# i8run/BigDL

Measured on AMD Instinct MI355X. Metric: images/sec (whole node) ResNet-50 224x224 bf16 at 1/2/4/8 MI355X, higher is better.
Workload: dtype bf16; 1 GPU; model=ResNet-50 v1.5 (BigDL ImageNet builder), global_batch=256, per_gpu_batch=256, image=224, parallelism=dp1, optimizer=SGD momentum 0.9 + L2 1e-4 (one rank: no gradient exchange), hip_graph=False, wgrad_side_stream=True, bucketed_overlap=False, grad_compress=none (no exchange)

## Files before the change

### bigdl_amd/nn/conv.py

```python
import math

import torch
import torch.nn.functional as F

from .. import ops
from ..ops import bn as bnops
from ..ops import conv as cv
from ..ops import conv_fn
from ..ops import side_stream
from .abstractnn import AutogradModule, TensorModule, _t_begin, _t_end
from .init_methods import RandomUniform, Zeros

CL = torch.channels_last
BF16 = torch.bfloat16


def _same_pad(inp, k, s, d=1):
    out = -(-inp // s)
    total = max((out - 1) * s + (k - 1) * d + 1 - inp, 0)
    return total // 2, total - total // 2


class SpatialConvolution(TensorModule):
    def __init__(self, nInputPlane, nOutputPlane, kernelW, kernelH, strideW=1, strideH=1, padW=0, padH=0,
# ... 188 lines not shown
        return y

    def _direct_groups(self):
        return self.nGroup > 1 and self.nInputPlane // self.nGroup <= 16

    def _geo_g(self, ph, pw):
        return [self.strideH, self.strideW, ph, pw, self.dilationH, self.dilationW, self.nGroup]

    def _fwd_gpu_grouped(self, x, ph, pw):
        G = self.nGroup
        cin, cout = self.nInputPlane // G, self.nOutputPlane // G
        if self._direct_groups():
            xf = x.float().contiguous()
            OH = cv.out_size(x.shape[2], self.kernelH, self.strideH, ph, self.dilationH)
            OW = cv.out_size(x.shape[3], self.kernelW, self.strideW, pw, self.dilationW)
            y = xf.new_empty(x.shape[0], self.nOutputPlane, OH, OW)
            ops.native.get().gconv(0, xf, self.weight.float().contiguous(),
                                   self.bias.float().contiguous() if self.bias is not None else None, y,
                                   self._geo_g(ph, pw))
            if self.fuse_relu:
                y.relu_()
            self._xf = xf
            self._geom = (x.shape, ph, pw)
            return y.to(BF16).contiguous(memory_format=CL)
        outs = []
        w = self.weight
        self._x16 = cv.to_nhwc_bf16(x) if x.shape[1] % 8 == 0 else None
        for g in range(G):
            xg = cv.to_nhwc_bf16(x[:, g * cin:(g + 1) * cin].contiguous(memory_format=CL))
            wg = cv.weight_krsc_bf16(w[g * cout:(g + 1) * cout])
            bg = self.bias[g * cout:(g + 1) * cout] if self.bias is not None else None
            outs.append(cv.conv2d_fwd(xg, wg, bg, (self.strideH, self.strideW), (ph, pw),
                                      (self.dilationH, self.dilationW), relu=self.fuse_relu))
        self._geom = (x.shape, ph, pw)
        return torch.cat(outs, dim=1).contiguous(memory_format=CL)

    def updateGradInput(self, input, gradOutput):
        if not self.propagateBack:
            return None
        x = self._nchw(input)
        gy = self._nchw(gradOutput)
        squeeze = x.dim() == 3
        if squeeze:
            x, gy = x.unsqueeze(0), gy.unsqueeze(0)
        H, W = x.shape[2], x.shape[3]
        x, ph, pw, eh, ew = self._prep(x)
        if gy.is_cuda:
            gy = self._relu_mask(gy)
            once = getattr(self, "_dgrad_bn_once", False)
            self._dgrad_bn_once = False
            bn_src = getattr(input, "_bn_bwd", None) if (getattr(self, "_dgrad_bn_ok", False) or once) else None
            if bn_src is not None and not torch.is_tensor(bn_src[4]):
                bn_src = bn_src[:4] + ((input if bn_src[4] else None),)
            gi = self._dgrad_gpu(x, gy, ph, pw, None if (squeeze or eh or ew or self.format != "NCHW") else bn_src)
        else:
            gy = self._relu_mask(gy)
            gi = torch.nn.grad.conv2d_input(x.shape, self.weight, gy.float(), (self.strideH, self.strideW),
                                            (ph, pw), (self.dilationH, self.dilationW), self.nGroup)
        if eh or ew:
            gi = gi[:, :, :H, :W]
            if gi.is_cuda:
                gi = gi.contiguous(memory_format=CL)
        if squeeze:
            gi = gi.squeeze(0)
        return self._fmt_out(gi)

    def _relu_mask(self, gy):
        if not self.fuse_relu:
            return gy
        if gy.is_cuda and gy.dtype == BF16:
            return ops.relu_bwd_gpu(gy.contiguous(memory_format=CL), self.output)
        return gy * (self.output > 0)

    def _dgrad_gpu(self, x, gy, ph, pw, bn_src=None):
        gy16 = gy if (gy.dtype == BF16 and gy.is_contiguous(memory_format=CL)) else gy.to(BF16, memory_format=CL)
        if self.nGroup == 1:
            w16 = self._w16_padded()
            if gy16.shape[1] % 8:
                gy16 = cv.pad_dim(gy16, 1)
                w16 = cv.pad_dim(w16, 0)
            wt = getattr(self, "_wt_cache", None)
            if getattr(self, "_wt_stamp", None) != cv.WT_STAMP[0] or wt is None or \
                    tuple(wt.shape) != (w16.shape[1], w16.shape[2], w16.shape[3], w16.shape[0]):
                wt = cv.transpose_w(w16)
            Cp = w16.shape[1]
            xs = (x.shape[0], Cp, x.shape[2], x.shape[3])
            addend = getattr(self, "_dgrad_addend", None)
            self._dgrad_addend = None
            addend_zm = None
            if isinstance(addend, tuple):
                addend, addend_zm = addend
            if addend is not None and Cp != x.shape[1]:
                raise RuntimeError("dgrad addend requires unpadded channels")
            bn = None
            if bn_src is not None and Cp == x.shape[1]:
                bnmod, bx, bmean, baff, bz = bn_src
                bzm = None
                if bz is not None and bz.dtype == torch.uint8:
                    bz, bzm = None, bz
                bn = {"x": bx, "z": bz, "zm": bzm, "mean": bmean, "aff": baff,
                      "red": bnops.new_stats(Cp, gy16.device)}
            gi = cv.conv2d_dgrad(gy16, wt, xs, (self.strideH, self.strideW), (ph, pw),
                                 (self.dilationH, self.dilationW), addend=addend, bn=bn, addend_zm=addend_zm)
            if Cp != x.shape[1]:
                gi = gi[:, : x.shape[1]].contiguous(memory_format=CL)
            elif bn is not None and bn.get("done"):
                gi._bn_red = (bnmod, bn["red"])
            return gi
        G = self.nGroup
        cin, cout = self.nInputPlane // G, self.nOutputPlane // G
        if self._direct_groups():
            gyf = gy.float().contiguous()
            dx = torch.empty(x.shape[0], self.nInputPlane, x.shape[2], x.shape[3], device=gy.device)
            ops.native.get().gconv(1, dx, self.weight.float().contiguous(), None, gyf, self._geo_g(ph, pw))
            return dx.to(BF16).contiguous(memory_format=CL)
        parts = []
        for g in range(G):
            wg = cv.pad_dim(cv.weight_krsc_bf16(self.weight[g * cout:(g + 1) * cout]), 0)
            gyg = cv.pad_dim(gy16[:, g * cout:(g + 1) * cout].contiguous(memory_format=CL), 1)
            xs = (x.shape[0], wg.shape[1], x.shape[2], x.shape[3])
            gi = cv.conv2d_dgrad(gyg, cv.transpose_w(wg), xs, (self.strideH, self.strideW), (ph, pw),
                                 (self.dilationH, self.dilationW))
            parts.append(gi[:, :cin])
        return torch.cat(parts, dim=1).contiguous(memory_format=CL)

    def backward(self, input, gradOutput):
        side = None if self._frozen else side_stream.stream_for(gradOutput)
        if side is None:
            return super().backward(input, gradOutput)
        t0 = _t_begin(gradOutput)
        self.gradInput = self.updateGradInput(input, gradOutput)
        side_stream.begin(side)
        with torch.cuda.stream(side):
            self.accGradParameters(input, gradOutput)
            self._apply_regularizers()
        side_stream.keep(side, input, gradOutput, self.output, getattr(self, "_x16", None),
                         *(getattr(self, "_xpair", None) or (None,))[:1])
        _t_end(self, t0, "backward_time")
        return self.gradInput

    def accGradParameters(self, input, gradOutput):
        x = self._nchw(input)
        gy = self._nchw(gradOutput)
        if x.dim() == 3:
            x, gy = x.unsqueeze(0), gy.unsqueeze(0)
        x, ph, pw, _, _ = self._prep(x)
        if gy.is_cuda:
            gy = self._relu_mask(gy) if self.fuse_relu and not getattr(self, "_masked_cached", False) else gy
            self._wgrad_gpu(x, gy, ph, pw)
            return
        gy = self._relu_mask(gy).float()
        gw = torch.nn.grad.conv2d_weight(x.float(), self.weight.shape, gy, (self.strideH, self.strideW), (ph, pw),
                                         (self.dilationH, self.dilationW), self.nGroup)
        self.gradWeight.add_(gw, alpha=self.scaleW)
        if self.bias is not None:
            self.gradBias.add_(gy.sum(dim=(0, 2, 3)), alpha=self.scaleB)
# ... 340 lines not shown
```

### bigdl_amd/nn/fusion.py

```python
import os

import torch

from ..utils.table import Table
from .activation import ReLU
from .containers import ConcatTable, Sequential, add_activity
from .conv import SpatialConvolution
from .linear import Linear
from .normalization import BatchNormalization
from .table_ops import CAddTable


_TRAIN_NODE_ATTRS = ("res_src", "pass_index", "fold_fanout", "fold_bn")


def _reset(m):
    from .graph import Graph

    for x in [m] + list(m.flattened_layers()):
        if isinstance(x, Graph) and getattr(x, "_order0", None) is not None:
            x.order = x._order0
            x._order0 = None
        if isinstance(x, Graph):
            for n in x.order:
# ... 132 lines not shown
    while isinstance(m, Sequential) and m.modules and m._residual_plan is None:
        m = m.modules[-1]
    return m


def _fuse_sequential(seq):
    mods = seq.modules
    if (len(mods) == 3 and isinstance(mods[0], ConcatTable) and len(mods[0].modules) == 2
            and isinstance(mods[1], CAddTable) and isinstance(mods[2], ReLU)):
        branch, short = mods[0].modules
        if isinstance(branch, Sequential) and branch.modules and isinstance(branch.modules[-1], BatchNormalization):
            bn = branch.modules[-1]
            if bn.nOutput % 8 == 0:
                bn.fuse_relu = True
                seq._residual_plan = (branch, short, bn)
    for a, b in zip(mods[:-1], mods[1:]):
        if isinstance(a, SpatialConvolution) and isinstance(b, BatchNormalization) and a.nGroup == 1:
            a.emit_stats = True
        elif isinstance(a, BatchNormalization) and isinstance(b, ReLU):
            a.fuse_relu = True
            b.passthrough = True
    for a, b, c in zip(mods[:-2], mods[1:-1], mods[2:]):
        if (_dgrad_bn_enabled() and isinstance(a, BatchNormalization) and a.fuse_relu and isinstance(b, ReLU) and b.passthrough
                and isinstance(c, SpatialConvolution) and c.nGroup == 1):
            c._dgrad_bn_ok = True
        elif isinstance(a, (SpatialConvolution, Linear)) and isinstance(b, ReLU):
            a.fuse_relu = True
            b.passthrough = True
    for a, b, c in zip(mods[:-2], mods[1:-1], mods[2:]):
        _plan_deferred_bn(a, b, c)


DEFER_LEVEL = [int(os.environ.get("BIGDL_BN_DEFER", "1") or 0)]


def _defer_consumer(c):
    from .pooling import SpatialMaxPooling

    if isinstance(c, SpatialConvolution):
        if DEFER_LEVEL[0] < 2:
            return False
        return (c.nGroup == 1 and c.format == "NCHW" and type(c).updateOutput is SpatialConvolution.updateOutput
                and type(c)._wgrad_gpu is SpatialConvolution._wgrad_gpu and c.kernelW == 3 and c.kernelH == 3
                and c.strideW == 1 and c.strideH == 1 and c.dilationW == 1 and c.dilationH == 1)
    return DEFER_LEVEL[0] >= 1 and type(c) is SpatialMaxPooling and c.format == "NCHW"


def _plan_deferred_bn(a, b, c):
    if (isinstance(a, BatchNormalization) and a.fuse_relu and not getattr(a, "_graph_dres", False)
            and isinstance(b, ReLU) and b.passthrough and _defer_consumer(c)):
        a._defer_ok = True


def residual_forward(seq, x):
    branch, short, bn = seq._residual_plan
    concat, add, relu = seq.modules
    res = short.forward(x)
    h = x
    for m in branch.modules[:-1]:
        h = m.forward(h)
    if tuple(res.shape) != tuple(h.shape[:1]) + (bn.nOutput,) + tuple(h.shape[2:]):
        raise ValueError(f"residual block: shortcut output {tuple(res.shape)} does not match the branch output")
    out = bn.updateOutput(h, residual=res)
    bn.output = out
    branch.output = out
    concat.output = Table(out, res)
    add.output = out
    relu.output = out
    seq._res_h = h
    return out


MASKED_ADDEND = [os.environ.get("BIGDL_MASKED_ADDEND", "1") != "0"]


SHORTCUT_BN_RED = [os.environ.get("BIGDL_SHORTCUT_BN_RED", "1") != "0"]


def _native_det():
    from ..ops import native

    return native.deterministic()


def residual_backward(seq, x, gradOutput):
    branch, short, bn = seq._residual_plan
    mods = branch.modules
    first = mods[0]
    can_fold = (isinstance(first, SpatialConvolution) and first.propagateBack and first.nGroup == 1
                and first.format == "NCHW" and first.nInputPlane % 8 == 0)
    masked = None
    zm = getattr(bn, "_zm", None)
    if (MASKED_ADDEND[0] and can_fold and zm is not None and type(short).__name__ == "Identity" and first.strideH == 1
            and first.strideW == 1 and torch.is_tensor(gradOutput) and gradOutput.is_cuda
            and tuple(gradOutput.shape) == tuple(x.shape) and x.dtype == torch.bfloat16):
        dh, _ = bn.backward_fused(seq._res_h, gradOutput, need_dres=False)
        gz = gradOutput
        if gz.dtype != torch.bfloat16 or not gz.is_contiguous(memory_format=torch.channels_last):
            gz = gz.to(torch.bfloat16).contiguous(memory_format=torch.channels_last)
        masked = (gz, zm)
        gs = None
    else:
        sec, sbn = None, None
        if SHORTCUT_BN_RED[0] and isinstance(short, Sequential) and short.modules:
            sbn = short.modules[-1]
            xs = getattr(sbn, "_xin", None)
            xb = getattr(bn, "_xin", None)
            if (isinstance(sbn, BatchNormalization) and sbn.train and not sbn.fuse_relu and xs is not None
                    and xb is not None and xs.is_cuda and xs.shape == xb.shape and xs.stride() == xb.stride()
                    and xs.dtype == torch.bfloat16 and xs.shape[1] % 8 == 0 and not _native_det()):
                from ..ops import bn as bnops

                sec = (xs, sbn.saveMean, bnops.new_stats(xs.shape[1], xs.device))
        dh, dres = bn.backward_fused(seq._res_h, gradOutput, need_dres=True, sec=sec)
        if sec is not None:
            dres._bn_red = (sbn, sec[2])
        gs = short.backward(x, dres)
    bn.gradInput = dh
    fold = masked is not None or (can_fold and gs is not None and gs.dtype == x.dtype and gs.shape == x.shape)
    g = dh
    for i in range(len(mods) - 2, -1, -1):
        inp = mods[i - 1].output if i > 0 else x
        if i == 0 and fold:
            first._dgrad_addend = masked if masked is not None else gs
            first._dgrad_bn_once = _dgrad_bn_enabled()
        g = mods[i].backward(inp, g)
    return g if fold else add_activity(g, gs)


def _graph_users(g):
    users = {}
    for n in g.order:
        for p in n.prevs:
            users.setdefault(p.id, []).append(n)
    return users


def _conv_fusable(n):
    m = n.element
    return (type(m).__name__ in ("SpatialConvolution", "SpatialShareConvolution", "SpatialDilatedConvolution")
            and isinstance(m, SpatialConvolution) and m.nGroup == 1 and m.format == "NCHW")


def _conv_out_shape(conv, x):
    from ..ops.conv import out_size

    N, _, H, W = x.shape
    ph, pw = conv._pads(H, W)
    return (N, conv.nOutputPlane, out_size(H, conv.kernelH, conv.strideH, ph, conv.dilationH),
            out_size(W, conv.kernelW, conv.strideW, pw, conv.dilationW))


def _topo_with_deps(g, extra):
    order, state = [], {}
    for root in list(g.output_nodes) + list(g.inputs_nodes):
        stack = [(root, False)]
        while stack:
            n, done = stack.pop()
            if done:
                if state.get(n.id) != 2:
                    state[n.id] = 2
                    order.append(n)
                continue
            st = state.get(n.id)
            if st == 2:
                continue
            if st == 1:
                raise ValueError("inference fusion created a cycle")
            state[n.id] = 1
            stack.append((n, True))
            for p in reversed(list(n.prevs) + extra.get(n.id, [])):
                if state.get(p.id) != 2:
# ... 154 lines not shown
```

### bigdl_amd/nn/normalization.py

```python
import math
import os

import torch
import torch.nn.functional as F

from .. import ops
from ..ops import bn as bnops
from .abstractnn import AutogradModule, TensorModule, _t_begin, _t_end
from .init_methods import Ones, RandomUniform, Zeros

_ZMASK = os.environ.get("BIGDL_BN_ZMASK", "1") != "0"
_DEFER = [os.environ.get("BIGDL_BN_DEFER", "1") != "0"]
CL = torch.channels_last
BF16 = torch.bfloat16


class BatchNormalization(TensorModule):

    def __init__(self, nOutput, eps=1e-5, momentum=0.1, affine=True, initWeight=None, initBias=None,
                 initGradWeight=None, initGradBias=None, dataFormat="NCHW"):
        super().__init__()
        self.nOutput = nOutput
        self.eps = eps
        self.momentum = momentum
# ... 13 lines not shown
        self.saveStd = None
        self.weightInitMethod = RandomUniform(0.0, 1.0) if affine else None
        self.biasInitMethod = Zeros()
        self.reset()
        if initWeight is not None and affine:
            self.weight.copy_(torch.as_tensor(initWeight))
        if initBias is not None and affine:
            self.bias.copy_(torch.as_tensor(initBias))
        if initGradWeight is not None and affine:
            self.gradWeight.copy_(torch.as_tensor(initGradWeight))
        if initGradBias is not None and affine:
            self.gradBias.copy_(torch.as_tensor(initGradBias))

    def reset(self):
        if self.affine:
            with torch.no_grad():
                self.weightInitMethod.init(self.weight)
                self.biasInitMethod.init(self.bias)
        self.runningMean.zero_()
        self.runningVar.fill_(1.0)

    def setParallism(self, n):
        from ..parallel.sync_bn import make_sync_fn

        self.sync_fn = make_sync_fn() if n and n > 1 else None
        return self

    def _to_nchw(self, x):
        if self.dataFormat == "NHWC" and x.dim() == 4:
            return x.permute(0, 3, 1, 2)
        return x

    def _from_nchw(self, y):
        if self.dataFormat == "NHWC" and y.dim() == 4:
            return y.permute(0, 2, 3, 1)
        return y

    def _gpu_ok(self, x):
        if not x.is_cuda or self.nOutput % 8 != 0:
            return False
        if x.dim() == 4:
            return True
        return x.dim() == 2

    def _prep_gpu(self, x):
        if x.dim() == 4:
            if x.dtype != BF16 or not x.is_contiguous(memory_format=CL):
                x = x.to(BF16, memory_format=CL)
        else:
            if x.dtype != BF16 or not x.is_contiguous():
                x = x.to(BF16).contiguous()
        return x

    def updateOutput(self, input, residual=None):
        if residual is None:
            residual = self.__dict__.pop("_graph_residual", None)
        x = self._to_nchw(input)
        if self._gpu_ok(x):
            stats = getattr(input, "_bn_stats", None) if self.train else None
            x = self._prep_gpu(x)
            res = residual
            if res is not None and (res.dtype != BF16 or res.stride() != x.stride()):
                res = res.to(BF16).contiguous(memory_format=CL if x.dim() == 4 else torch.contiguous_format)
            zm = None
            if self.train and self.fuse_relu and res is not None and x.shape[1] % 8 == 0 and _ZMASK:
                zm = torch.empty(x.numel() // 8, dtype=torch.uint8, device=x.device)
            if (self.train and self.fuse_relu and res is None and getattr(self, "_defer_ok", False) and _DEFER[0]
                    and x.dim() == 4 and self.dataFormat == "NCHW"):
                sm, si, aff = bnops.bn_prepare_gpu(x, self.weight, self.bias, self.runningMean, self.runningVar,
                                                   self.eps, self.momentum, stats=stats, sync_fn=self.sync_fn)
                self.saveMean, self.saveStd = sm, si
                self._aff, self._zm, self._xin = aff, None, x
                y = bnops.deferred(x, aff)
                y._bn_bwd = (self, x, sm, aff, False)
                return y
            y, sm, si, aff = bnops.bn_forward_gpu(x, self.weight, self.bias, self.runningMean, self.runningVar,
                                                   self.eps, self.momentum, self.train, stats=stats, res=res,
                                                   relu=self.fuse_relu, sync_fn=self.sync_fn if self.train else None,
                                                   zm=zm)
            self.saveMean, self.saveStd = sm, si
            self._aff = aff if (self.fuse_relu and res is None) else None
            self._zm = zm
            self._xin = x
            if self.train and self.fuse_relu:
                y._bn_bwd = (self, x, sm, self._aff, zm if zm is not None else res is not None)
            return self._from_nchw(y)
        xf = x.float()
        y, mean, invstd = bnops.bn_forward_cpu(xf, self.weight, self.bias, self.runningMean, self.runningVar, self.eps,
                                               self.momentum, self.train,
                                               sync_fn=self.sync_fn if self.train else None)
        if residual is not None:
            y = y + residual.float()
        if self.fuse_relu:
            y = torch.relu(y)
        self.saveMean, self.saveStd = mean, invstd
        self._xin = xf
        return self._from_nchw(y.to(input.dtype) if input.is_floating_point() else y)

    def _direct_grads(self):
        return (not self._frozen) and self.affine and self.scaleW == 1.0 and self.scaleB == 1.0

    def backward_fused(self, input, gradOutput, need_dres=False, sec=None):
        gz = self._to_nchw(gradOutput)
        x = self._xin
        if gz.dtype != BF16 or gz.stride() != x.stride():
            gz = gz.to(BF16).contiguous(memory_format=CL if x.dim() == 4 else torch.contiguous_format)
        aff = getattr(self, "_aff", None)
        zm = getattr(self, "_zm", None)
        z = self._to_nchw(self.output) if (self.fuse_relu and aff is None and zm is None) else None
        direct = self._direct_grads()
        dg = self.gradWeight if direct else (torch.zeros_like(self.runningMean) if self.affine else None)
        db = self.gradBias if direct else (torch.zeros_like(self.runningMean) if self.affine else None)
        pre = getattr(gradOutput, "_bn_red", None)
        red = pre[1] if (pre is not None and pre[0] is self and self.train) else None
        graph_res = getattr(self, "_graph_dres", False)
        dx, dres = bnops.bn_backward_gpu(gz, z, x, self.saveMean, self.saveStd, self.weight, dg, db,
                                         training=self.train, need_dres=need_dres or graph_res,
                                         sync_fn=self.sync_fn if self.train else None, aff=aff, red=red, zm=zm,
                                         sec=sec)
        if graph_res:
            self._dres = dres
        if not direct and self.affine and not self._frozen:
            self.gradWeight.add_(dg, alpha=self.scaleW)
            self.gradBias.add_(db, alpha=self.scaleB)
        return self._from_nchw(dx), dres

    def backward(self, input, gradOutput):
        t0 = _t_begin(gradOutput)
        x = self._to_nchw(input)
        if self._gpu_ok(x):
            self.gradInput, _ = self.backward_fused(input, gradOutput)
        else:
            self.gradInput = self.updateGradInput(input, gradOutput)
            if not self._frozen:
                self.accGradParameters(input, gradOutput)
        _t_end(self, t0, "backward_time")
        return self.gradInput

    def _cpu_grads(self, gradOutput):
# ... 183 lines not shown
```

### bigdl_amd/ops/bn.py

```python
import os
import torch

from . import native


def _P(x):
    return x.numel() // x.shape[1]


def stat_slots():
    return native.get().STAT_SLOTS


class _StatsArena:

    def __init__(self):
        self.buf, self.off, self.active, self.need = None, 0, False, 0

    def begin(self, device):
        if self.need and (self.buf is None or self.buf.numel() < self.need or self.buf.device != device):
            self.buf = torch.empty(self.need, dtype=torch.float32, device=device)
        if self.buf is not None:
            if self.buf.is_cuda and int(os.environ.get("BIGDL_NATIVE_FILL", "7")) & 2:
                native.get().fill_bytes(self.buf, 0)
            else:
                self.buf.zero_()
        self.off, self.need, self.active = 0, 0, True

    def end(self):
        self.active = False

    def take(self, n, device):
        n_al = (n + 63) // 64 * 64
        self.need += n_al
        if self.active and self.buf is not None and self.buf.device == device and self.off + n_al <= self.buf.numel():
            t = self.buf[self.off:self.off + n]
            self.off += n_al
            return t
        t = torch.empty(n, dtype=torch.float32, device=device)
        if t.is_cuda:
            native.get().fill_bytes(t, 0)
            return t
        return t.zero_()


ARENA = _StatsArena()


def new_stats(C, device):
    return ARENA.take(stat_slots() * 2 * C, torch.device(device))


def _reduce_slots_for_sync(buf, C, P, sync_fn):
    red = torch.empty(2 * C, dtype=torch.float32, device=buf.device)
    native.get().bn_slot_reduce(buf, stat_slots(), C, red)
    P = sync_fn(red, P)
    return red, 1, P


def bn_forward_gpu(x, gamma, beta, rmean, rvar, eps, momentum, training, stats=None, res=None, relu=False,
                   out=None, sync_fn=None, zm=None):
    C = x.shape[1]
    P = _P(x)
    C_ = native.get()
    dev = x.device
    if out is None:
        out = torch.empty_like(x)
    aff = torch.empty(2 * C, dtype=torch.float32, device=dev)
    scale, shift = aff[:C], aff[C:]
    smean = torch.empty(C, dtype=torch.float32, device=dev)
    sinv = torch.empty(C, dtype=torch.float32, device=dev)
    nslots = stat_slots()
    Ptot = P
    if training:
        if stats is None:
            stats = new_stats(C, dev)
            C_.bn_stats(x, stats, P, C)
        if sync_fn is not None:
            stats, nslots, Ptot = _reduce_slots_for_sync(stats, C, P, sync_fn)
    else:
        stats, nslots = scale, 0
    C_.bn_finalize(stats, nslots, gamma, beta, rmean, rvar, smean, sinv, scale, shift, Ptot, C, float(eps),
                   float(momentum), bool(training))
    C_.bn_apply(x, scale, shift, res, out, P, C, bool(relu), zm)
    return out, smean, sinv, aff


def bn_prepare_gpu(x, gamma, beta, rmean, rvar, eps, momentum, stats=None, sync_fn=None):
    C = x.shape[1]
    P = _P(x)
    C_ = native.get()
    dev = x.device
    aff = torch.empty(2 * C, dtype=torch.float32, device=dev)
    smean = torch.empty(C, dtype=torch.float32, device=dev)
    sinv = torch.empty(C, dtype=torch.float32, device=dev)
    nslots, Ptot = stat_slots(), P
    if stats is None:
        stats = new_stats(C, dev)
        C_.bn_stats(x, stats, P, C)
    if sync_fn is not None:
        stats, nslots, Ptot = _reduce_slots_for_sync(stats, C, P, sync_fn)
    C_.bn_finalize(stats, nslots, gamma, beta, rmean, rvar, smean, sinv, aff[:C], aff[C:], Ptot, C, float(eps),
                   float(momentum), True)
    return smean, sinv, aff


def deferred(x, aff):
    y = x.detach()
    y._bn_pre = aff
    return y


def materialize(t):
    aff = getattr(t, "_bn_pre", None)
    if aff is None:
        return t
    C = t.shape[1]
    y = torch.empty_like(t)
    native.get().bn_apply(t, aff[:C], aff[C:], None, y, _P(t), C, True)
    return y


def bn_backward_gpu(dz, z, x, smean, sinv, gamma, dgamma, dbeta, training=True, need_dres=False, need_dx=True,
                    sync_fn=None, aff=None, red=None, zm=None, sec=None):
    C = x.shape[1]
    P = _P(x)
    C_ = native.get()
    nslots, Ptot = 0, P
    if not training:
        red = None
    elif red is None:
        red = new_stats(C, x.device)
        C_.bn_bwd_reduce(dz, z, x, smean, red, P, C, aff, zm)
    if training:
        nslots = stat_slots()
        if sync_fn is not None:
            red, nslots, Ptot = _reduce_slots_for_sync(red, C, P, sync_fn)
    coef = torch.empty(3 * C, dtype=torch.float32, device=x.device)
    dx = torch.empty_like(x) if need_dx else None
    dres = torch.empty_like(x) if need_dres else None
    if sec is not None and dres is not None and training:
        x2, mean2, red2 = sec
        C_.bn_bwd_apply(dz, z, x, smean, sinv, gamma, red, nslots, coef, dx, dres, dgamma, dbeta, Ptot, C, aff, zm,
                        x2=x2, mean2=mean2, red2=red2)
    else:
        C_.bn_bwd_apply(dz, z, x, smean, sinv, gamma, red, nslots, coef, dx, dres, dgamma, dbeta, Ptot, C, aff, zm)
    return dx, dres


def bn_forward_cpu(x, gamma, beta, rmean, rvar, eps, momentum, training, sync_fn=None):
    dims = [0] + list(range(2, x.dim()))
    shape = [1, -1] + [1] * (x.dim() - 2)
    if training:
        n = x.numel() // x.shape[1]
        if sync_fn is not None:
            buf = torch.cat([x.sum(dim=dims), (x * x).sum(dim=dims)]).double()
            n = sync_fn(buf, n)
            C = x.shape[1]
            mean = (buf[:C] / n).float()
            var = (buf[C:] / n - (buf[:C] / n) ** 2).clamp_min(0).float()
        else:
            mean = x.mean(dim=dims)
            var = x.var(dim=dims, unbiased=False)
        if rmean is not None:
            unb = var * n / max(n - 1, 1)
            rmean.mul_(1 - momentum).add_(momentum * mean)
            rvar.mul_(1 - momentum).add_(momentum * unb)
    else:
        mean, var = rmean, rvar
    invstd = torch.rsqrt(var + eps)
    xhat = (x - mean.view(shape)) * invstd.view(shape)
    y = xhat
# ... 25 lines not shown
```

### bigdl_amd/ops/conv.py

```python
import os
import torch
import torch.nn.functional as F

from . import native

CL = torch.channels_last
BF16 = torch.bfloat16


def out_size(inp, k, s, p, d=1, ceil=False):
    eff = d * (k - 1) + 1
    num = inp + 2 * p - eff
    if ceil:
        o = -(-num // s) + 1
        if (o - 1) * s >= inp + p:
            o -= 1
        return o
    return num // s + 1


def to_nhwc_bf16(x, cpad=8):
    N, C, H, W = x.shape
    Cp = -(-C // cpad) * cpad
    if x.dtype == BF16 and Cp == C and x.is_contiguous(memory_format=CL):
# ... 56 lines not shown
        native.get().bn_stats(dense, stats, N * OH * OW, K)
        return (out, mat) if pre is not None else out
    mat = native.get().conv_nt(x, w16, out, bias, stats, geo, _fwd_taps(R, S, ph, pw, dh, dw), relu, addend, pre=pre)
    return (out, mat) if pre is not None else out


_TAP_CACHE = {}


def _fwd_taps(R, S, ph, pw, dh, dw):
    key = ("f", R, S, ph, pw, dh, dw)
    t = _TAP_CACHE.get(key)
    if t is None:
        t = []
        for r in range(R):
            for s in range(S):
                t += [r * dh - ph, s * dw - pw, r * S + s]
        _TAP_CACHE[key] = t
    return t


def _fwd_geo(N, H, W, C, OH, OW, sh, sw, ldw, K):
    return [N, H, W, C, OH, OW, sh, sw, ldw, K, K, OH, OW, 1, 1, 0, 0]


def dgrad_phases(H, W, R, S, stride, pad, dil):
    sh, sw = stride
    ph, pw = pad
    dh, dw = dil
    key = ("d", H, W, R, S, sh, sw, ph, pw, dh, dw)
    res = _TAP_CACHE.get(key)
    if res is not None:
        return res
    res = []
    for a in range(sh):
        for b in range(sw):
            nI, nJ = -(-(H - a) // sh), -(-(W - b) // sw)
            if nI <= 0 or nJ <= 0:
                continue
            taps = []
            for r in range(R):
                if (a + ph - r * dh) % sh:
                    continue
                for s in range(S):
                    if (b + pw - s * dw) % sw:
                        continue
                    taps += [(a + ph - r * dh) // sh, (b + pw - s * dw) // sw, r * S + s]
            if taps:
                res.append((a, b, nI, nJ, taps))
    _TAP_CACHE[key] = res
    return res


def conv2d_dgrad(dy, w16t, x_shape, stride, pad, dil=(1, 1), out=None, addend=None, bn=None, addend_zm=None):
    N, C, H, W = x_shape
    _, K, OH, OW = dy.shape
    R, S = w16t.shape[1], w16t.shape[2]
    phases = dgrad_phases(H, W, R, S, stride, pad, dil)
    covered = sum(nI * nJ for (_, _, nI, nJ, _) in phases)
    if addend is not None and not addend.is_contiguous(memory_format=CL):
        addend = addend.contiguous(memory_format=CL)
    if out is None:
        out = torch.empty((N, C, H, W), dtype=BF16, device=dy.device, memory_format=CL)
    if addend_zm is not None and (addend is None or covered != H * W):
        raise ValueError("conv2d_dgrad: a masked addend needs an addend and a data gradient that covers every pixel")
    if covered != H * W:
        mask = 0
        for (a, b, _, _, _) in phases:
            mask |= 1 << (a * stride[1] + b)
        if (out.is_contiguous(memory_format=CL) and C % 8 == 0 and stride[0] * stride[1] <= 32
                and int(os.environ.get("BIGDL_NATIVE_FILL", "7")) & 4):
            native.get().dgrad_fill(out, addend, stride[0], stride[1], mask)
        elif addend is not None:
            out.copy_(addend)
        else:
            out.zero_()
    C_ = native.get()
    ldw = R * S * K
    bnk = {}
    if bn is not None and (covered == H * W or addend is None) and bn["x"].shape == out.shape \
            and bn["x"].stride() == out.stride() and not native.deterministic():
        bnk = dict(bn_x=bn["x"], bn_z=bn["z"], bn_mean=bn["mean"], bn_aff=bn["aff"], bn_red=bn["red"],
                   bn_zm=bn.get("zm"))
        bn["done"] = True
    for (a, b, nI, nJ, taps) in phases:
        geo = [N, OH, OW, K, nI, nJ, 1, 1, ldw, C, C, H, W, stride[0], stride[1], a, b]
        C_.conv_nt(dy, w16t, out, None, None, geo, taps, False, addend, addend_zm=addend_zm, **bnk)
    return out


WT_STAMP = [0]
_DESC_CACHE = {}
DESC_BUILDS = [0]


def prepare_dgrad_weights(convs):
    WT_STAMP[0] += 1
    rows, mods, tile = [], [], 0
    for m in convs:
        if not getattr(m, "_w16_managed", False):
            continue
        wf = getattr(m, "weight", None)
        if wf is None or wf.dim() != 4 or wf.shape[0] % 8 or wf.shape[1] % 8:
            continue
        w16 = m._w16_padded()
        K, C, R, S = w16.shape
        if K % 8 or C % 8 or not w16.is_cuda or not w16.is_contiguous(memory_format=CL):
            continue
        if mods and w16.device != mods[0]._wt_cache.device:
            continue
        wt = getattr(m, "_wt_cache", None)
        if wt is None or tuple(wt.shape) != (C, R, S, K) or wt.device != w16.device:
            wt = torch.empty((C, R, S, K), dtype=BF16, device=w16.device)
            m._wt_cache = wt
        rows.append((w16.data_ptr(), wt.data_ptr(), K, R * S, C, tile))
        tile += ((C + 31) // 32) * ((K + 31) // 32) * R * S
        mods.append(m)
    if not rows:
        return 0
    key = tuple(rows)
    desc = _DESC_CACHE.get(key)
    if desc is None:
        if torch.cuda.is_current_stream_capturing():
            return 0
        if len(_DESC_CACHE) > 8:
            _DESC_CACHE.clear()
        desc = torch.tensor(rows, dtype=torch.int64).to(mods[0]._wt_cache.device)
        _DESC_CACHE[key] = desc
        DESC_BUILDS[0] += 1
    native.get().transpose_krsc_batched(desc, len(rows), tile)
    for m in mods:
        m._wt_stamp = WT_STAMP[0]
    return len(rows)


def end_dgrad_weights():
    WT_STAMP[0] += 1


def transpose_w(w16, out=None):
# ... 149 lines not shown
```

### csrc/batchnorm.hip

```cpp
#include "common.h"
#include "kernels.h"
#include <stdlib.h>

#define STAT_SLOTS BIGDL_STAT_SLOTS

namespace {

template <int MODE, int U>
__global__ __launch_bounds__(256) void chan_reduce_kernel(const bf16_t* __restrict__ x, const bf16_t* __restrict__ dz,
                                                          const bf16_t* __restrict__ z, const float* __restrict__ mean,
                                                          float* __restrict__ out, long P, int C, long rows_per_block,
                                                          const float* __restrict__ aff, const uint8_t* __restrict__ zm) {
  __shared__ float sm[256 * 16];
  const int G = C >> 3;
  const int tid = threadIdx.x;
  const long rbeg = blockIdx.x * rows_per_block;
  const long rend = min(P, rbeg + rows_per_block);
  for (int gbase = 0; gbase < G; gbase += 256) {
    const int gcount = min(256, G - gbase);
    const int rpi = 256 / gcount;
    const int g = gbase + tid % gcount, rsub = tid / gcount;
    float a1[8], a2[8], mu[8], sc[8], sh[8];
#pragma unroll
    for (int e = 0; e < 8; ++e) { a1[e] = 0.f; a2[e] = 0.f; mu[e] = 0.f; sc[e] = 0.f; sh[e] = 0.f; }
// ... 50 lines not shown
              a1[2 * e] += dl; a1[2 * e + 1] += dh;
              a2[2 * e] += dl * (xl - mu[2 * e]);
              a2[2 * e + 1] += dh * (xh - mu[2 * e + 1]);
            }
          }
        }
      }
    }
#pragma unroll
    for (int e = 0; e < 8; ++e) { sm[tid * 16 + e] = a1[e]; sm[tid * 16 + 8 + e] = a2[e]; }
    __syncthreads();
    for (int w = tid; w < gcount * 16; w += 256) {
      const int gg = w >> 4, slot = w & 15;
      float t = 0.f;
      for (int rs = 0; rs < rpi; ++rs) t += sm[(rs * gcount + gg) * 16 + slot];
      const int ch = (gbase + gg) * 8 + (slot & 7);
      atomicAdd(out + (size_t)(blockIdx.x & (STAT_SLOTS - 1)) * 2 * C + (slot < 8 ? 0 : C) + ch, t);
    }
    __syncthreads();
  }
}

int bn_unroll() {
  static int u = [] {
    const char* e = getenv("BIGDL_BN_UNROLL");
    const int v = e ? atoi(e) : 4;
    return (v == 1 || v == 2 || v == 8) ? v : 4;
  }();
  return u;
}

__device__ __forceinline__ void slot_sums(const float* __restrict__ red, int nslots, int C, int c, int sl, double& s1,
                                          double& s2) {
  s1 = 0.0;
  s2 = 0.0;
  for (int k = sl; k < nslots; k += 32) {
    s1 += red[(size_t)k * 2 * C + c];
    s2 += red[(size_t)k * 2 * C + C + c];
  }
#pragma unroll
  for (int o = 16; o > 0; o >>= 1) {
    s1 += __shfl_xor(s1, o, 64);
    s2 += __shfl_xor(s2, o, 64);
  }
}

__global__ void bn_finalize_kernel(const float* __restrict__ stats, int nslots, const float* __restrict__ gamma,
                                   const float* __restrict__ beta, float* run_mean, float* run_var, float* save_mean,
                                   float* save_invstd, float* scale, float* shift, long P, int C, float eps,
                                   float momentum, int training) {
  const int lane = threadIdx.x & 63, sl = lane & 31;
  const int c = (blockIdx.x * (blockDim.x >> 6) + (threadIdx.x >> 6)) * 2 + (lane >> 5);
  if (c >= C) return;
  float mean, invstd;
  if (training) {
    double s1, s2;
    slot_sums(stats, nslots, C, c, sl, s1, s2);
    if (sl != 0) return;
    mean = (float)(s1 / (double)P);
    const float var = fmaxf((float)(s2 / (double)P - (double)mean * mean), 0.f);
    invstd = rsqrtf(var + eps);
    save_mean[c] = mean;
    save_invstd[c] = invstd;
    if (run_mean) {
      const float unbiased = P > 1 ? var * (float)P / (float)(P - 1) : var;
      run_mean[c] = momentum * mean + (1.f - momentum) * run_mean[c];
      run_var[c] = momentum * unbiased + (1.f - momentum) * run_var[c];
    }
  } else {
    if (sl != 0) return;
    mean = run_mean[c];
    invstd = rsqrtf(run_var[c] + eps);
    if (save_mean) { save_mean[c] = mean; save_invstd[c] = invstd; }
  }
  const float g = gamma ? gamma[c] : 1.f, b = beta ? beta[c] : 0.f;
  scale[c] = g * invstd;
  shift[c] = b - mean * g * invstd;
}

template <int U>
__global__ __launch_bounds__(256) void bn_apply_kernel(const bf16_t* __restrict__ x, const float* __restrict__ scale,
                                                       const float* __restrict__ shift, const bf16_t* __restrict__ res,
                                                       bf16_t* __restrict__ y, long P, int C, long rpb, int relu,
                                                       uint8_t* __restrict__ zm) {
  const int G = C >> 3;
  const int gbase = blockIdx.y * 256;
  const int gcount = min(256, G - gbase);
  const int rpi = 256 / gcount;
  const int g = gbase + threadIdx.x % gcount, rsub = threadIdx.x / gcount;
  if (rsub >= rpi) return;
  const long rbeg = blockIdx.x * rpb, rend = min(P, rbeg + rpb);
  const int c0 = g * 8;
  const v4f s0 = *reinterpret_cast<const v4f*>(scale + c0), s1 = *reinterpret_cast<const v4f*>(scale + c0 + 4);
  const v4f b0 = *reinterpret_cast<const v4f*>(shift + c0), b1 = *reinterpret_cast<const v4f*>(shift + c0 + 4);
  const float sc[8] = {s0[0], s0[1], s0[2], s0[3], s1[0], s1[1], s1[2], s1[3]};
  const float sh[8] = {b0[0], b0[1], b0[2], b0[3], b1[0], b1[1], b1[2], b1[3]};
  for (long r0 = rbeg + rsub; r0 < rend; r0 += (long)U * rpi) {
    v4u vx[U], vr[U];
#pragma unroll
    for (int u = 0; u < U; ++u) {
      const long r = r0 + (long)u * rpi;
      const long i = (r < rend ? r : rbeg) * G + g;
      vx[u] = reinterpret_cast<const v4u*>(x)[i];
      vr[u] = v4u{0u, 0u, 0u, 0u};
      if (res) vr[u] = reinterpret_cast<const v4u*>(res)[i];
    }
#pragma unroll
    for (int u = 0; u < U; ++u) {
      const long r = r0 + (long)u * rpi;
      v4u o;
#pragma unroll
      for (int e = 0; e < 4; ++e) {
        float l = lo_bf(vx[u][e]) * sc[2 * e] + sh[2 * e];
        float h = hi_bf(vx[u][e]) * sc[2 * e + 1] + sh[2 * e + 1];
        if (res) { l += lo_bf(vr[u][e]); h += hi_bf(vr[u][e]); }
        if (relu) { l = fmaxf(l, 0.f); h = fmaxf(h, 0.f); }
        o[e] = pack2bf(l, h);
      }
      if (r < rend) {
        reinterpret_cast<v4u*>(y)[r * G + g] = o;
        if (zm) zm[r * G + g] = (uint8_t)bf_to_mask8(o);
      }
    }
  }
}

__global__ void bn_bwd_coeff_kernel(const float* __restrict__ red, int nslots, const float* __restrict__ mean,
                                    const float* __restrict__ invstd, const float* __restrict__ gamma,
                                    float* __restrict__ coef, float* dgamma, float* dbeta, long P, int C, int training) {
  const int lane = threadIdx.x & 63, sl = lane & 31;
  const int c = (blockIdx.x * (blockDim.x >> 6) + (threadIdx.x >> 6)) * 2 + (lane >> 5);
  if (c >= C) return;
  double sdy = 0.0, sdyx = 0.0;
  if (training) slot_sums(red, nslots, C, c, sl, sdy, sdyx);
  if (sl != 0) return;
  const float is = invstd[c];
  const float g = gamma ? gamma[c] : 1.f;
  float A = g * is, B = 0.f, D = 0.f;
  if (training) {
    const float mdy = (float)(sdy / (double)P);
    const float mdyx = (float)(sdyx / (double)P) * is;
    B = -g * is * is * mdyx;
    D = g * is * (mean[c] * is * mdyx - mdy);
    if (dgamma) dgamma[c] += (float)sdyx * is;
    if (dbeta) dbeta[c] += (float)sdy;
  }
  coef[c] = A; coef[C + c] = B; coef[2 * C + c] = D;
}

__global__ void bn_slot_reduce_kernel(const float* __restrict__ in, int nslots, int C, float* __restrict__ out) {
  const int c = blockIdx.x * blockDim.x + threadIdx.x;
  if (c >= 2 * C) return;
  float t = 0.f;
  for (int k = 0; k < nslots; ++k) t += in[(size_t)k * 2 * C + c];
  out[c] = t;
}

__device__ __forceinline__ void load8(const float* p, float* v) {
  const v4f a = *reinterpret_cast<const v4f*>(p), b = *reinterpret_cast<const v4f*>(p + 4);
  v[0] = a[0]; v[1] = a[1]; v[2] = a[2]; v[3] = a[3]; v[4] = b[0]; v[5] = b[1]; v[6] = b[2]; v[7] = b[3];
}

template <int U, bool R2>
__global__ __launch_bounds__(256) void bn_bwd_apply_kernel(const bf16_t* __restrict__ dz, const bf16_t* __restrict__ z,
                                                           const bf16_t* __restrict__ x, const float* __restrict__ coef,
                                                           bf16_t* __restrict__ dx, bf16_t* __restrict__ dres, long P,
                                                           int C, long rpb, const float* __restrict__ aff,
                                                           const uint8_t* __restrict__ zm, const bf16_t* __restrict__ x2,
                                                           const float* __restrict__ mean2, float* __restrict__ red2) {
  const int G = C >> 3;
  const bool xmask = z == nullptr && zm == nullptr && aff != nullptr;
  const __amdgpu_buffer_rsrc_t rzm = __builtin_amdgcn_make_buffer_rsrc(
      const_cast<uint8_t*>(zm), (short)0, zm ? (int)min(P * C / 8, 0x7fffffffl) : 0, 0x00020000);
  const bf16_t* zp = (z && !zm) ? z : x;
  const int gbase = blockIdx.y * 256;
  const int gcount = min(256, G - gbase);
  const int rpi = 256 / gcount;
  const int g = gbase + threadIdx.x % gcount, rsub = threadIdx.x / gcount;
  if (!R2 && rsub >= rpi) return;
  const long rbeg = blockIdx.x * rpb, rend = rsub < rpi ? min(P, rbeg + rpb) : rbeg;
  const int c0 = g * 8;
  float A[8], B[8], D[8], S[8], T[8], M2[8], a1[8], a2[8];
  load8(coef + c0, A);
  load8(coef + C + c0, B);
  load8(coef + 2 * C + c0, D);
  if (xmask) {
    load8(aff + c0, S);
    load8(aff + C + c0, T);
  }
  if (R2) {
    load8(mean2 + c0, M2);
#pragma unroll
    for (int e = 0; e < 8; ++e) { a1[e] = 0.f; a2[e] = 0.f; }
  }
  for (long r0 = rbeg + rsub; r0 < rend; r0 += (long)U * rpi) {
    v4u vd[U], vz[U], vx[U], vx2[U];
    unsigned zb[U];
#pragma unroll
    for (int u = 0; u < U; ++u) {
      const long r = r0 + (long)u * rpi;
      const long i = (r < rend ? r : rbeg) * G + g;
      vd[u] = reinterpret_cast<const v4u*>(dz)[i];
      zb[u] = __builtin_amdgcn_raw_buffer_load_b8(rzm, (unsigned)i, 0, 0);
      vz[u] = reinterpret_cast<const v4u*>(zp)[i];
      vx[u] = reinterpret_cast<const v4u*>(x)[i];
      if (R2) vx2[u] = reinterpret_cast<const v4u*>(x2)[i];
    }
#pragma unroll
    for (int u = 0; u < U; ++u)
      vz[u] = zm ? mask8_to_bf(zb[u]) : z ? vz[u] : v4u{0xffffffffu, 0xffffffffu, 0xffffffffu, 0xffffffffu};
#pragma unroll
    for (int u = 0; u < U; ++u) {
      const long r = r0 + (long)u * rpi;
// ... 56 lines not shown
}

int grid_for(long work, int per_block, int cap) {
  long g = (work + per_block - 1) / per_block;
  if (g > cap) g = cap;
  if (g < 1) g = 1;
  return (int)g;
}

void launch_reduce(int mode, const bf16_t* x, const bf16_t* dz, const bf16_t* z, const float* mean, float* out, long P,
                   int C, hipStream_t st, const float* aff = nullptr, const uint8_t* zm = nullptr) {
  const int G = C >> 3;
  const int rpi = 256 / (G < 256 ? G : 256);
  long blocks = (P + rpi * 16 - 1) / (rpi * 16);
  if (blocks > 2048) blocks = 2048;
  if (bigdl_deterministic() && blocks > 2 * STAT_SLOTS) blocks = 2 * STAT_SLOTS;
  if (blocks < 1) blocks = 1;
  const long rpb = (P + blocks - 1) / blocks;
  blocks = (P + rpb - 1) / rpb;
#define BN_RED(M, U) chan_reduce_kernel<M, U><<<(int)blocks, 256, 0, st>>>(x, dz, z, mean, out, P, C, rpb, aff, zm)
  if (mode == 0) { aff = nullptr; zm = nullptr; }
  switch (bn_unroll()) {
    case 1: if (mode == 0) BN_RED(0, 1); else BN_RED(1, 1); break;
    case 2: if (mode == 0) BN_RED(0, 2); else BN_RED(1, 2); break;
    case 8: if (mode == 0) BN_RED(0, 8); else BN_RED(1, 8); break;
    default: if (mode == 0) BN_RED(0, 4); else BN_RED(1, 4); break;
  }
#undef BN_RED
}

}

extern "C" {

void bigdl_bn_stats(const uint16_t* x, float* stats, long P, int C, hipStream_t st) {
  launch_reduce(0, x, nullptr, nullptr, nullptr, stats, P, C, st);
  HIP_LAUNCH_CHECK();
}

void bigdl_bn_finalize(const float* stats, int nslots, const float* gamma, const float* beta, float* run_mean,
                       float* run_var, float* save_mean, float* save_invstd, float* scale, float* shift, long P, int C,
                       float eps, float momentum, int training, hipStream_t st) {
  bn_finalize_kernel<<<(C + 7) / 8, 256, 0, st>>>(stats, nslots, gamma, beta, run_mean, run_var, save_mean,
                                                   save_invstd, scale, shift, P, C, eps, momentum, training);
  HIP_LAUNCH_CHECK();
}

void bigdl_bn_slot_reduce(const float* in, int nslots, int C, float* out, hipStream_t st) {
  bn_slot_reduce_kernel<<<(2 * C + 255) / 256, 256, 0, st>>>(in, nslots, C, out);
  HIP_LAUNCH_CHECK();
}

void bigdl_bn_apply(const uint16_t* x, const float* scale, const float* shift, const uint16_t* res, uint16_t* y,
                    long P, int C, int relu, hipStream_t st, uint8_t* zm) {
  long rpb = 0;
  const dim3 grid = stationary_grid(P, C, &rpb);
  switch (bn_unroll()) {
    case 1: bn_apply_kernel<1><<<grid, 256, 0, st>>>(x, scale, shift, res, y, P, C, rpb, relu, zm); break;
    case 2: bn_apply_kernel<2><<<grid, 256, 0, st>>>(x, scale, shift, res, y, P, C, rpb, relu, zm); break;
    case 8: bn_apply_kernel<8><<<grid, 256, 0, st>>>(x, scale, shift, res, y, P, C, rpb, relu, zm); break;
    default: bn_apply_kernel<4><<<grid, 256, 0, st>>>(x, scale, shift, res, y, P, C, rpb, relu, zm); break;
  }
  HIP_LAUNCH_CHECK();
}

void bigdl_bn_bwd_reduce(const uint16_t* dz, const uint16_t* z, const uint16_t* x, const float* mean, float* red,
                         long P, int C, const float* aff, hipStream_t st, const uint8_t* zm) {
  launch_reduce(1, x, dz, z, mean, red, P, C, st, aff, zm);
  HIP_LAUNCH_CHECK();
}

void bigdl_bn_bwd_apply(const uint16_t* dz, const uint16_t* z, const uint16_t* x, const float* mean,
                        const float* invstd, const float* gamma, const float* red, int nslots, float* coef,
                        uint16_t* dx, uint16_t* dres, float* dgamma, float* dbeta, long P, int C, int training,
                        const float* aff, hipStream_t st, const uint8_t* zm, const uint16_t* x2u,
                        const float* mean2, float* red2) {
  const bf16_t* x2 = reinterpret_cast<const bf16_t*>(x2u);
  bn_bwd_coeff_kernel<<<(C + 7) / 8, 256, 0, st>>>(red, nslots, mean, invstd, gamma, coef, dgamma, dbeta, P, C,
                                                    training);
  if (dx || dres) {
    long rpb = 0;
    const dim3 grid = stationary_grid(P, C, &rpb);
    if (red2) {
#define BWD2(UU) bn_bwd_apply_kernel<UU, true><<<grid, 256, 0, st>>>(dz, z, x, coef, dx, dres, P, C, rpb, aff, zm, x2, mean2, red2)
      switch (bn_unroll()) {
        case 1: BWD2(1); break;
        case 2: BWD2(2); break;
        case 8: BWD2(8); break;
        default: BWD2(4); break;
      }
#undef BWD2
    } else {
#define BWD1(UU) bn_bwd_apply_kernel<UU, false><<<grid, 256, 0, st>>>(dz, z, x, coef, dx, dres, P, C, rpb, aff, zm, nullptr, nullptr, nullptr)
      switch (bn_unroll()) {
        case 1: BWD1(1); break;
        case 2: BWD1(2); break;
        case 8: BWD1(8); break;
        default: BWD1(4); break;
      }
#undef BWD1
    }
  }
  HIP_LAUNCH_CHECK();
}

}
```

### csrc/bindings.cpp

```cpp
#include <torch/extension.h>
#include <ATen/hip/HIPContext.h>
#include <vector>
#include <algorithm>
#include "kernels.h"

namespace {

using at::Tensor;
using OptT = c10::optional<Tensor>;

hipStream_t stream() { return at::hip::getCurrentHIPStream().stream(); }

void check(const Tensor& t, at::ScalarType dt, const char* name) {
  TORCH_CHECK(t.is_cuda(), name, " must be a GPU tensor");
  TORCH_CHECK(t.scalar_type() == dt, name, " has dtype ", t.scalar_type(), ", expected ", dt);
}
const uint16_t* cbf(const Tensor& t, const char* n) { check(t, at::kBFloat16, n); return (const uint16_t*)t.data_ptr(); }
uint16_t* mbf(const Tensor& t, const char* n) { check(t, at::kBFloat16, n); return (uint16_t*)t.data_ptr(); }
const float* cf(const Tensor& t, const char* n) { check(t, at::kFloat, n); return (const float*)t.data_ptr(); }
float* mf(const Tensor& t, const char* n) { check(t, at::kFloat, n); return (float*)t.data_ptr(); }
const uint16_t* ocbf(const OptT& t, const char* n) { return (t && t->defined()) ? cbf(*t, n) : nullptr; }
uint16_t* ombf(const OptT& t, const char* n) { return (t && t->defined()) ? mbf(*t, n) : nullptr; }
const float* ocf(const OptT& t, const char* n) { return (t && t->defined()) ? cf(*t, n) : nullptr; }
float* omf(const OptT& t, const char* n) { return (t && t->defined()) ? mf(*t, n) : nullptr; }
uint8_t* omzm(const OptT& t, int64_t P, int64_t C, const char* n) {
  if (!(t && t->defined())) return nullptr;
  check(*t, at::kByte, n);
  TORCH_CHECK(t->is_contiguous() && t->numel() == P * (C / 8), n, ": sign mask must be a contiguous [P][C/8] uint8 tensor");
  return (uint8_t*)t->data_ptr();
}

OptT conv_nt(const Tensor& src, const Tensor& wt, const Tensor& out, const OptT& bias, const OptT& stats,
             std::vector<int64_t> geo, std::vector<int64_t> taps, bool relu, const OptT& addend, const OptT& bn_x,
             const OptT& bn_z, const OptT& bn_mean, const OptT& bn_aff, const OptT& bn_red, bool accumulate,
             const OptT& bn_zm, const OptT& addend_zm, const OptT& pre) {
  TORCH_CHECK(geo.size() == 17 || geo.size() == 18, "conv_nt: bad geometry");
  if (stats && stats->defined())
    TORCH_CHECK(stats->numel() >= BIGDL_STAT_SLOTS * 2 * geo[9], "conv_nt: stats must hold STAT_SLOTS x 2Ncol");
  TORCH_CHECK(taps.size() % 3 == 0 && !taps.empty() && taps.size() / 3 <= CONV_MAX_TAPS, "conv_nt: bad taps");
  TORCH_CHECK(!bigdl_deterministic() || (!(stats && stats->defined()) && !(bn_red && bn_red->defined())),
              "conv_nt: epilogue statistics are not deterministic; use bn_stats in deterministic mode");
  ConvArgs a;
  a.src = cbf(src, "src"); a.wt = cbf(wt, "wt");
  a.out = nullptr; a.out32 = nullptr; a.accum32 = accumulate ? 1 : 0;
  if (out.scalar_type() == at::kFloat) a.out32 = mf(out, "out");
  else a.out = mbf(out, "out");
  a.bias = ocf(bias, "bias"); a.stats = omf(stats, "stats");
  a.addend = ocbf(addend, "addend");
  if (a.addend) TORCH_CHECK(addend->numel() == out.numel(), "conv_nt: addend must match out");
  a.bnx = ocbf(bn_x, "bn_x"); a.bnz = ocbf(bn_z, "bn_z"); a.bnmean = ocf(bn_mean, "bn_mean");
  a.bnaff = ocf(bn_aff, "bn_aff"); a.bnred = omf(bn_red, "bn_red");
  a.addzm = nullptr;
  if (addend_zm && addend_zm->defined()) {
    TORCH_CHECK(a.addend && geo[10] == geo[9] && geo[9] % 8 == 0, "conv_nt: a masked addend needs ldo == Ncol");
    a.addzm = omzm(addend_zm, out.numel() / geo[9], geo[9], "addend_zm");
  }
  a.bnzm = nullptr;
  if (bn_zm && bn_zm->defined()) {
    TORCH_CHECK(geo[10] == geo[9] && geo[9] % 8 == 0, "conv_nt: a sign-mask z needs a dense output (ldo == Ncol)");
    a.bnzm = omzm(bn_zm, out.numel() / geo[9], geo[9], "bn_zm");
  }
  if (a.bnred) {
    TORCH_CHECK(a.bnx && a.bnmean && bn_x->numel() == out.numel(), "conv_nt: bn_x must match out, bn_mean required");
    TORCH_CHECK(!a.bnz || bn_z->numel() == out.numel(), "conv_nt: bn_z must match out");
    TORCH_CHECK(bn_mean->numel() >= geo[9] && (!a.bnaff || bn_aff->numel() >= 2 * geo[9]), "conv_nt: bn vectors");
    TORCH_CHECK(bn_red->numel() >= BIGDL_STAT_SLOTS * 2 * geo[9], "conv_nt: bn_red must hold STAT_SLOTS x 2Ncol");
  }
  a.Nb = geo[0]; a.Hs = geo[1]; a.Ws = geo[2]; a.Cs = geo[3]; a.OH = geo[4]; a.OW = geo[5];
  a.mul_h = geo[6]; a.mul_w = geo[7]; a.ldw = geo[8]; a.Ncol = geo[9]; a.ldo = geo[10];
  a.OHo = geo[11]; a.OWo = geo[12]; a.omul_h = geo[13]; a.omul_w = geo[14]; a.ooff_h = geo[15]; a.ooff_w = geo[16];
  a.pstride = geo.size() == 18 ? (int)geo[17] : 0;
  TORCH_CHECK(a.pstride >= 0 && a.pstride % 8 == 0, "conv_nt: pixel stride must be a multiple of 8");
  a.pre = ocf(pre, "pre");
  if (a.pre)
    TORCH_CHECK(pre->numel() >= 2 * geo[3] && a.pstride == 0 && src.numel() % geo[3] == 0 &&
                    (src.is_contiguous() || src.is_contiguous(at::MemoryFormat::ChannelsLast)),
                "conv_nt: pre must hold 2 x Cs floats for a dense source");
  a.ntaps = (int)(taps.size() / 3);
  a.Kdim = a.ntaps * a.Cs;
  a.M = a.Nb * a.OH * a.OW;
  a.ident_out = (a.OHo == a.OH && a.OWo == a.OW && a.omul_h == 1 && a.omul_w == 1 && a.ooff_h == 0 && a.ooff_w == 0);
  a.relu = relu ? 1 : 0;
  int max_tk = 0;
  for (int t = 0; t < a.ntaps; ++t) {
    a.tap_h[t] = (short)taps[3 * t]; a.tap_w[t] = (short)taps[3 * t + 1]; a.tap_k[t] = (short)taps[3 * t + 2];
    max_tk = std::max(max_tk, (int)a.tap_k[t]);
  }
  if (a.pstride > 0) {
    int max_tw = 0;
    for (int t = 0; t < a.ntaps; ++t) max_tw = std::max(max_tw, (int)a.tap_w[t]);
    TORCH_CHECK(((int64_t)(a.OW - 1) * a.mul_w + max_tw) * a.pstride + a.Cs <= (int64_t)a.Ws * a.pstride,
                "conv_nt: a window crosses its source row");
    TORCH_CHECK(src.numel() >= (int64_t)a.Nb * a.Hs * a.Ws * a.pstride, "conv_nt: src too small");
  } else {
    TORCH_CHECK(src.numel() >= (int64_t)a.Nb * a.Hs * a.Ws * a.Cs, "conv_nt: src too small");
  }
  TORCH_CHECK(wt.numel() >= (int64_t)(a.Ncol - 1) * a.ldw + (int64_t)(max_tk + 1) * a.Cs, "conv_nt: weight too small");
  const int64_t out_avail = (int64_t)(out.storage().nbytes() / out.element_size()) - out.storage_offset();
  TORCH_CHECK(a.ldo >= a.Ncol && out_avail >= ((int64_t)a.Nb * a.OHo * a.OWo - 1) * a.ldo + a.Ncol,
              "conv_nt: out too small");
  if (a.addend) TORCH_CHECK(a.ldo == a.Ncol, "conv_nt: an addend needs a dense output (ldo == Ncol)");
  TORCH_CHECK((a.OH - 1) * a.omul_h + a.ooff_h < a.OHo && (a.OW - 1) * a.omul_w + a.ooff_w < a.OWo,
              "conv_nt: output placement out of range");
  OptT materialised;
  if (a.pre && !bigdl_conv_pre_applies(&a)) {
    Tensor y = at::empty_like(src);
    const int64_t P = src.numel() / a.Cs;
    bigdl_bn_apply(a.src, a.pre, a.pre + a.Cs, nullptr, (uint16_t*)y.data_ptr(), P, a.Cs, 1, stream(), nullptr);
    a.src = (const uint16_t*)y.data_ptr();
    a.pre = nullptr;
    materialised = y;
  }
  a.ws = nullptr;
  Tensor ws;
  const long wsn = bigdl_conv_nt_plan(&a);
  if (wsn > 0) {
    ws = at::empty({wsn}, out.options().dtype(at::kFloat));
    a.ws = ws.data_ptr<float>();
  }
  const int rc = bigdl_conv_nt(&a, stream());
  TORCH_CHECK(rc == 0, "conv_nt: unsupported shape (channels must be a multiple of 8; fp32 output needs Ncol % 8 "
              "== 0 and no fused stats / BN / ReLU / addend)");
  return materialised;
}

void conv_wgrad(const Tensor& dy, const Tensor& src, const Tensor& dw, const OptT& dbias, std::vector<int64_t> geo,
                const OptT& pre) {
  TORCH_CHECK(geo.size() == 18, "conv_wgrad: bad geometry");
  WgradArgs a;
  a.dy = cbf(dy, "dy"); a.src = cbf(src, "src"); a.dw = mf(dw, "dw"); a.dbias = omf(dbias, "dbias");
  int* f = &a.Nb;
  for (int i = 0; i < 18; ++i) f[i] = (int)geo[i];
  a.m_per_split = 0;
  a.ws = nullptr;
  a.splits = 0;
  a.pre = ocf(pre, "pre");
  Tensor det_ws;
  a.det_ws = nullptr;
  if (bigdl_deterministic() && a.dbias) {
    det_ws = at::empty({(int64_t)BIGDL_DET_SLOTS * a.Ncol}, dw.options().dtype(at::kFloat));
    a.det_ws = det_ws.data_ptr<float>();
  }
  Tensor mat;
  if (a.pre) {
    TORCH_CHECK(pre->numel() >= 2 * a.Cs && src.numel() % a.Cs == 0, "conv_wgrad: pre must hold 2 x Cs floats");
    if (!bigdl_wgrad_pre_applies(&a)) {
      mat = at::empty_like(src);
      bigdl_bn_apply(a.src, a.pre, a.pre + a.Cs, nullptr, (uint16_t*)mat.data_ptr(), src.numel() / a.Cs, a.Cs, 1,
                     stream(), nullptr);
      a.src = (const uint16_t*)mat.data_ptr();
      a.pre = nullptr;
    }
  }
  TORCH_CHECK(dw.numel() >= (int64_t)a.Ncol * a.Kdim, "conv_wgrad: dw too small");
  TORCH_CHECK(a.M == a.Nb * a.OH * a.OW, "conv_wgrad: M mismatch");
  TORCH_CHECK(dy.numel() >= (int64_t)(a.M - 1) * a.ldy + a.Ncol, "conv_wgrad: dy too small");
  TORCH_CHECK(src.numel() >= (int64_t)a.Nb * a.Hs * a.Ws * a.Cs, "conv_wgrad: src too small");
  Tensor ws;
  const long wsn = bigdl_conv_wgrad_plan(&a);
  if (wsn > 0) {
    ws = at::empty({wsn}, dw.options().dtype(at::kFloat));
    a.ws = ws.data_ptr<float>();
  }
  const int rc = bigdl_conv_wgrad(&a, stream());
  TORCH_CHECK(rc == 0, "conv_wgrad: unsupported shape (channels must be a multiple of 8)");
}

bool conv_wgrad_uses_p8(std::vector<int64_t> geo, bool bias) {
  TORCH_CHECK(geo.size() == 18, "conv_wgrad_uses_p8: bad geometry");
  WgradArgs a{};
  int* f = &a.Nb;
  for (int i = 0; i < 18; ++i) f[i] = (int)geo[i];
  static float dummy;
  a.dbias = bias ? &dummy : nullptr;
  return bigdl_conv_wgrad_uses_p8(&a) != 0;
}

void transpose_krsc(const Tensor& w, const Tensor& wt, int64_t K, int64_t RS, int64_t C) {
  TORCH_CHECK(w.numel() == K * RS * C && wt.numel() == K * RS * C, "transpose_krsc: size mismatch");
  bigdl_transpose_krsc(cbf(w, "w"), mbf(wt, "wt"), (int)K, (int)RS, (int)C, stream());
}

void bn_stats(const Tensor& x, const Tensor& stats, int64_t P, int64_t C) {
  TORCH_CHECK(C % 8 == 0 && x.numel() == P * C, "bn_stats: shape");
  TORCH_CHECK(stats.numel() >= BIGDL_STAT_SLOTS * 2 * C, "bn_stats: stats must hold STAT_SLOTS x 2C");
  bigdl_bn_stats(cbf(x, "x"), mf(stats, "stats"), P, (int)C, stream());
}
void bn_finalize(const Tensor& stats, int64_t nslots, const OptT& gamma, const OptT& beta, const OptT& rmean,
                 const OptT& rvar, const OptT& smean, const OptT& sinv, const Tensor& scale, const Tensor& shift,
                 int64_t P, int64_t C, double eps, double momentum, bool training) {
  TORCH_CHECK(stats.numel() >= nslots * 2 * C, "bn_finalize: stats size");
  bigdl_bn_finalize(cf(stats, "stats"), (int)nslots, ocf(gamma, "gamma"), ocf(beta, "beta"), omf(rmean, "rmean"),
                    omf(rvar, "rvar"), omf(smean, "smean"), omf(sinv, "sinv"), mf(scale, "scale"),
                    mf(shift, "shift"), P, (int)C, (float)eps, (float)momentum, training ? 1 : 0, stream());
}
void bn_slot_reduce(const Tensor& in, int64_t nslots, int64_t C, const Tensor& out) {
  TORCH_CHECK(in.numel() >= nslots * 2 * C && out.numel() >= 2 * C, "bn_slot_reduce: size");
  bigdl_bn_slot_reduce(cf(in, "in"), (int)nslots, (int)C, mf(out, "out"), stream());
}
void bn_apply(const Tensor& x, const Tensor& scale, const Tensor& shift, const OptT& res, const Tensor& y, int64_t P,
              int64_t C, bool relu, const OptT& zm) {
  TORCH_CHECK(C % 8 == 0 && x.numel() == P * C && y.numel() == P * C, "bn_apply: shape");
  bigdl_bn_apply(cbf(x, "x"), cf(scale, "scale"), cf(shift, "shift"), ocbf(res, "res"), mbf(y, "y"), P, (int)C,
                 relu ? 1 : 0, stream(), omzm(zm, P, C, "zm"));
}
void bn_bwd_reduce(const Tensor& dz, const OptT& z, const Tensor& x, const Tensor& mean, const Tensor& red, int64_t P,
                   int64_t C, const OptT& aff, const OptT& zm) {
  TORCH_CHECK(C % 8 == 0 && x.numel() == P * C && dz.numel() == P * C, "bn_bwd_reduce: shape");
  TORCH_CHECK(red.numel() >= BIGDL_STAT_SLOTS * 2 * C, "bn_bwd_reduce: red must hold STAT_SLOTS x 2C");
  if (aff && aff->defined()) TORCH_CHECK(aff->numel() >= 2 * C && aff->is_contiguous(), "bn_bwd_reduce: aff is [2C]");
  bigdl_bn_bwd_reduce(cbf(dz, "dz"), ocbf(z, "z"), cbf(x, "x"), cf(mean, "mean"), mf(red, "red"), P, (int)C,
                      ocf(aff, "aff"), stream(), omzm(zm, P, C, "zm"));
}
void bn_bwd_apply(const Tensor& dz, const OptT& z, const Tensor& x, const Tensor& mean, const Tensor& invstd,
                  const OptT& gamma, const OptT& red, int64_t nslots, const Tensor& coef, const OptT& dx,
                  const OptT& dres, const OptT& dgamma, const OptT& dbeta, int64_t P, int64_t C, const OptT& aff,
                  const OptT& zm, const OptT& x2, const OptT& mean2, const OptT& red2) {
  TORCH_CHECK(coef.numel() >= 3 * C, "bn_bwd_apply: coef size");
  const bool r2 = red2 && red2->defined();
  if (r2) {
    TORCH_CHECK(dres && dres->defined() && x2 && x2->defined() && mean2 && mean2->defined(),
                "bn_bwd_apply: red2 needs dres, x2 and mean2");
    TORCH_CHECK(x2->numel() == x.numel() && x2->strides() == x.strides(), "bn_bwd_apply: x2 must match x's layout");
    TORCH_CHECK(mean2->numel() >= C && red2->numel() >= (int64_t)BIGDL_STAT_SLOTS * 2 * C, "bn_bwd_apply: mean2 / red2 size");
  }
  if (aff && aff->defined()) TORCH_CHECK(aff->numel() >= 2 * C && aff->is_contiguous(), "bn_bwd_apply: aff is [2C]");
  const bool training = red && red->defined();
  bigdl_bn_bwd_apply(cbf(dz, "dz"), ocbf(z, "z"), cbf(x, "x"), cf(mean, "mean"), cf(invstd, "invstd"),
                     ocf(gamma, "gamma"), ocf(red, "red"), (int)nslots, mf(coef, "coef"), ombf(dx, "dx"),
                     ombf(dres, "dres"), omf(dgamma, "dgamma"), omf(dbeta, "dbeta"), P, (int)C, training ? 1 : 0,
                     ocf(aff, "aff"), stream(), omzm(zm, P, C, "zm"), r2 ? cbf(*x2, "x2") : nullptr,
                     r2 ? cf(*mean2, "mean2") : nullptr, r2 ? omf(red2, "red2") : nullptr);
}

void dgrad_fill(const Tensor& out, const OptT& addend, int64_t sh, int64_t sw, int64_t mask) {
  TORCH_CHECK(out.dim() == 4 && out.is_contiguous(at::MemoryFormat::ChannelsLast) && out.size(1) % 8 == 0,
              "dgrad_fill: out must be NHWC bf16 with C % 8 == 0");
  TORCH_CHECK(sh * sw <= 32, "dgrad_fill: at most 32 stride phases");
  if (addend && addend->defined())
    TORCH_CHECK(addend->sizes() == out.sizes() && addend->is_contiguous(at::MemoryFormat::ChannelsLast),
                "dgrad_fill: addend must match out (NHWC)");
  bigdl_dgrad_fill(mbf(out, "out"), ocbf(addend, "addend"), out.size(0) * out.size(2) * out.size(3), out.size(2),
                   out.size(3), out.size(1), (int)sh, (int)sw, (unsigned)mask, stream());
}
void hog_cus(int64_t n, double us, const Tensor& done) {
  TORCH_CHECK(done.is_cuda() && done.scalar_type() == at::kInt && done.numel() >= n, "hog_cus: done must be int32 cuda [n]");
  bigdl_hog_cus((int)n, us, done.data_ptr<int>(), stream());
}
void spin_us(double us, const Tensor& done) {
  TORCH_CHECK(done.is_cuda() && done.scalar_type() == at::kInt && done.numel() >= 1, "spin_us: done must be int32 cuda");
  bigdl_spin_us(us, done.data_ptr<int>(), stream());
}
void relu_fwd(const Tensor& x, const Tensor& y) {
  TORCH_CHECK(x.numel() == y.numel(), "relu: size");
  bigdl_relu_fwd(cbf(x, "x"), mbf(y, "y"), x.numel(), stream());
}
void relu_bwd(const Tensor& dy, const Tensor& y, const Tensor& dx) {
// ... 1074 lines not shown
                    ws.defined() ? ws.data_ptr<float>() : nullptr);
}
int64_t rows_of(const OptT& t, int64_t B, int64_t cols, const char* name) {
  if (!(t && t->defined())) return 0;
  TORCH_CHECK(t->dim() == 2 && t->size(0) == B && t->size(1) >= cols && t->stride(1) == 1, name,
              ": expected [B, >=", cols, "] rows with unit inner stride");
  return t->stride(0);
}
void need_flat(const OptT& t, int64_t n, const char* name) {
  if (t && t->defined()) TORCH_CHECK(t->is_contiguous() && t->numel() == n, name, ": expected ", n, " contiguous elements");
}
void gru_step(int64_t mode, const OptT& A, const Tensor& W, int64_t B, int64_t H, const OptT& xg, const OptT& hprev,
              const OptT& r, const OptT& z, const OptT& n, const OptT& rh16, const OptT& hout, const OptT& h16out,
              const OptT& dout, const OptT& dhp, const OptT& dx, const OptT& dn16, const OptT& drz16, const OptT& dh0) {
  TORCH_CHECK(W.dim() == 2 && W.is_contiguous(), "gru_step: W must be [N, K] contiguous");
  const int64_t N = W.size(0), K = W.size(1);
  TORCH_CHECK(H % 32 == 0 && K % 32 == 0 && N % 16 == 0 && B > 0, "gru_step: H, K multiples of 32, N of 16");
  TORCH_CHECK(mode >= 0 && mode <= 4, "gru_step: bad mode");
  TORCH_CHECK(N == (mode == 0 ? 2 * H : H) && K == (mode == 2 || mode == 4 ? 2 * H : H), "gru_step: W shape vs mode");
  GruStepArgs a{};
  a.mode = (int)mode; a.B = (int)B; a.H = (int)H; a.K = (int)K; a.N = (int)N;
  a.W = cbf(W, "W");
  if (A && A->defined()) { a.lda = rows_of(A, B, K, "A"); a.A = cbf(*A, "A"); }
  need_flat(r, B * H, "r"); need_flat(z, B * H, "z"); need_flat(n, B * H, "n"); need_flat(rh16, B * H, "rh16");
  need_flat(h16out, B * H, "h16out"); need_flat(dhp, B * H, "dhp"); need_flat(dn16, B * H, "dn16");
  need_flat(drz16, B * 2 * H, "drz16"); need_flat(dh0, B * H, "dh0");
  a.ldx = rows_of(xg, B, 3 * H, "xg"); a.ldhp = rows_of(hprev, B, H, "hprev"); a.ldho = rows_of(hout, B, H, "hout");
  a.ldd = rows_of(dout, B, H, "dout"); a.lddx = rows_of(dx, B, 3 * H, "dx");
  a.xg = ocf(xg, "xg"); a.hprev = ocf(hprev, "hprev"); a.r = omf(r, "r"); a.z = omf(z, "z"); a.n = omf(n, "n");
  a.rh16 = ombf(rh16, "rh16"); a.hout = omf(hout, "hout"); a.h16out = ombf(h16out, "h16out"); a.dout = ocf(dout, "dout");
  a.dhp = omf(dhp, "dhp"); a.dx = omf(dx, "dx"); a.dn16 = ombf(dn16, "dn16"); a.drz16 = ombf(drz16, "drz16");
  a.dh0 = omf(dh0, "dh0");
  switch (mode) {
    case 0: TORCH_CHECK(a.xg && a.r && a.z && a.rh16, "gru_step fwd r/z: xg, r, z, rh16 required"); break;
    case 1: TORCH_CHECK(a.A && a.xg && a.z && a.n && a.hout && a.h16out, "gru_step fwd n: A, xg, z, n, hout, h16out required"); break;
    case 2: TORCH_CHECK(a.z && a.n && a.dhp && a.dx && a.dn16 && a.drz16, "gru_step bwd h: z, n, dhp, dx, dn16, drz16 required"); break;
    case 3: TORCH_CHECK(a.A && a.r && a.dhp && a.dx && a.drz16, "gru_step bwd r: A, r, dhp, dx, drz16 required"); break;
    default: TORCH_CHECK(a.dhp && a.dh0, "gru_step bwd h0: dhp, dh0 required"); break;
  }
  TORCH_CHECK(bigdl_gru_step(&a, stream()) == 0, "gru_step: unsupported shape");
}

}

void register_host_runtime(pybind11::module& m);

PYBIND11_MODULE(TORCH_EXTENSION_NAME, m) {
  register_host_runtime(m);
  m.doc() = "bigdl_amd native HIP kernels for gfx950 (MI355X)";
  m.def("conv_nt", &conv_nt, py::arg("src"), py::arg("wt"), py::arg("out"), py::arg("bias"), py::arg("stats"),
        py::arg("geo"), py::arg("taps"), py::arg("relu"), py::arg("addend") = py::none(), py::arg("bn_x") = py::none(),
        py::arg("bn_z") = py::none(), py::arg("bn_mean") = py::none(), py::arg("bn_aff") = py::none(),
        py::arg("bn_red") = py::none(), py::arg("accumulate") = false, py::arg("bn_zm") = py::none(),
        py::arg("addend_zm") = py::none(), py::arg("pre") = py::none());
  m.def("conv_wgrad", &conv_wgrad, py::arg("dy"), py::arg("src"), py::arg("dw"), py::arg("dbias"), py::arg("geo"),
        py::arg("pre") = py::none());
  m.def("transpose_krsc", &transpose_krsc);
  m.def("bn_stats", &bn_stats);
  m.def("bn_finalize", &bn_finalize);
  m.def("bn_apply", &bn_apply, py::arg("x"), py::arg("scale"), py::arg("shift"), py::arg("res"), py::arg("y"),
        py::arg("P"), py::arg("C"), py::arg("relu"), py::arg("zm") = py::none());
  m.def("bn_slot_reduce", &bn_slot_reduce);
  m.attr("STAT_SLOTS") = BIGDL_STAT_SLOTS;
  m.def("bn_bwd_reduce", &bn_bwd_reduce, py::arg("dz"), py::arg("z"), py::arg("x"), py::arg("mean"), py::arg("red"),
        py::arg("P"), py::arg("C"), py::arg("aff") = py::none(), py::arg("zm") = py::none());
  m.def("bn_bwd_apply", &bn_bwd_apply, py::arg("dz"), py::arg("z"), py::arg("x"), py::arg("mean"), py::arg("invstd"),
        py::arg("gamma"), py::arg("red"), py::arg("nslots"), py::arg("coef"), py::arg("dx"), py::arg("dres"),
        py::arg("dgamma"), py::arg("dbeta"), py::arg("P"), py::arg("C"), py::arg("aff") = py::none(),
        py::arg("zm") = py::none(), py::arg("x2") = py::none(), py::arg("mean2") = py::none(),
        py::arg("red2") = py::none());
  m.def("relu_fwd", &relu_fwd);
  m.def("dgrad_fill", &dgrad_fill);
  m.def("maxpool_bwd_bnred", &maxpool_bwd_bnred, "k3 s2 maxpool backward + the producing BN's backward reduction",
        py::arg("dy"), py::arg("idx"), py::arg("dx"), py::arg("g"), py::arg("bx"), py::arg("mean"), py::arg("aff"),
        py::arg("zm"), py::arg("red"));
  m.def("hog_cus", &hog_cus, "n one-wave workgroups holding a whole CU's LDS each, spinning `us` microseconds");
  m.def("spin_us", &spin_us, "device-side delay of `us` microseconds on the current stream (straggler injection)");
  m.def("relu_bwd", &relu_bwd);
  m.def("add_bf16", &add_bf16);
  m.def("nchw_to_nhwc", &nchw_to_nhwc);
  m.def("nchw_to_pairs", &nchw_to_pairs);
  m.def("bmm_nt", &bmm_nt, py::arg("a"), py::arg("b"), py::arg("c"), py::arg("alpha") = 1.0, py::arg("accum") = false);
  m.def("pair_weight", &pair_weight);
  m.def("pair_wgrad_add", &pair_wgrad_add);
  m.def("tensor_apply", &tensor_apply, py::arg("out"), py::arg("a"), py::arg("b"), py::arg("c"), py::arg("size"),
        py::arg("so"), py::arg("sa"), py::arg("sb"), py::arg("sc"), py::arg("op"), py::arg("s0") = 0.0,
        py::arg("s1") = 0.0, py::arg("contiguous") = false);
  m.def("tensor_reduce", &tensor_reduce, py::arg("x"), py::arg("outer"), py::arg("R"), py::arg("inner"), py::arg("op"),
        py::arg("p"), py::arg("out"), py::arg("outi"), py::arg("mean"), py::arg("ws"), py::arg("chunks"));
  m.def("gemm_f32", &gemm_f32);
  m.def("index_op", &index_op);
  m.def("masked_fill", &masked_fill);
  m.def("mask_blocks", &mask_blocks);
  m.def("mask_scan", &mask_scan);
  m.def("mask_write", &mask_write);
  m.def("topk_f32", &topk_f32);
  m.def("gemv_f32", &gemv_f32);
  m.def("fill_bytes", &fill_bytes);
  m.def("gemm_bf16", &gemm_bf16, py::arg("a"), py::arg("b"), py::arg("out"), py::arg("form"), py::arg("alpha") = 1.0,
        py::arg("beta") = 0.0, py::arg("bias") = py::none(), py::arg("colsum") = py::none(), py::arg("colscale") = 1.0,
        py::arg("ws") = py::none());
  m.def("gemm_bf16_ws_bytes", &gemm_bf16_ws_bytes);
  m.def("copy_rows_i8", &copy_rows_i8);
  m.def("cast_f32_bf16", &cast_f32_bf16);
  m.def("cast_bf16_f32", &cast_bf16_f32);
  m.def("maxpool_fwd", &maxpool_fwd, py::arg("x"), py::arg("y"), py::arg("idx"), py::arg("g"), py::arg("pre") = py::none());
  m.def("maxpool_bwd", &maxpool_bwd);
  m.def("avgpool_fwd", &avgpool_fwd);
  m.def("avgpool_bwd", &avgpool_bwd);
  m.def("softmax_xent", &softmax_xent);
  m.def("sgd_step", &sgd_step, py::arg("w"), py::arg("g"), py::arg("mom"), py::arg("w16"), py::arg("lr"), py::arg("wd"), py::arg("momentum"), py::arg("dampening"), py::arg("nesterov"), py::arg("first"), py::arg("lr_dev") = py::none(), py::arg("seg_off") = py::none(), py::arg("seg_wd") = py::none(), py::arg("base") = 0);
  m.def("adam_step", &adam_step);
  m.def("optim_step", &optim_step);
  m.def("sumsq", &sumsq);
// ... 104 lines not shown
```

### csrc/conv_epilogue.h

```cpp
#pragma once
#include "common.h"
#include "kernels.h"

namespace {

struct GemmRowMap {
  __device__ __forceinline__ long operator()(const ConvArgs& a, int m) const {
    if (m >= a.M) return -1;
    if (a.ident_out) return m;
    const int ohw = a.OH * a.OW;
    const int nb = m / ohw, rem = m - nb * ohw;
    const int oh = rem / a.OW, ow = rem - oh * a.OW;
    return ((long)nb * a.OHo + oh * a.omul_h + a.ooff_h) * a.OWo + ow * a.omul_w + a.ooff_w;
  }
};

template <int MI, int NI, int TM, int TN, int NH = 1, int PAIR = 0, int NWM = 2, class RowMap = GemmRowMap>
__device__ __forceinline__ void nt_epilogue_lds(const ConvArgs& a, v4f (&acc)[MI][NI], int mbase, int nbase,
                                                int lane, int bid, float* wl, int wm = 0, RowMap rowmap = {}) {
  constexpr int GR = TN / 4;
  constexpr int LPR = TN / 8;
  constexpr int PPI = 64 / LPR;
  static_assert(TN % 8 == 0 && 64 % LPR == 0, "tile");
  auto gpos = [](int p, int g) { return (p * GR + (g ^ (p & (GR - 1)))) * 4; };
  const int q = lane % LPR;
  const int n = nbase + q * 8;
  const bool nok = n < a.Ncol;
  float bs[8];
#pragma unroll
  for (int e = 0; e < 8; ++e) bs[e] = (a.bias && nok) ? a.bias[n + e] : 0.f;
  float s1[8], s2[8];
#pragma unroll
  for (int e = 0; e < 8; ++e) s1[e] = s2[e] = 0.f;
  float bmu[8], bsc[8], bsh[8];
#pragma unroll
  for (int e = 0; e < 8; ++e) {
    const bool on = a.bnred && !a.stats && nok;
    bmu[e] = on ? a.bnmean[n + e] : 0.f;
    bsc[e] = (on && a.bnaff) ? a.bnaff[n + e] : 0.f;
    bsh[e] = (on && a.bnaff) ? a.bnaff[a.Ncol + n + e] : 0.f;
  }
  constexpr int NR = TM / PPI;
  constexpr int MIH = MI / NH, NRH = NR / NH;
  static_assert(MI % NH == 0 && NR % NH == 0, "row chunks");
  const bool bnw = a.bnred && !a.stats;
#pragma unroll
  for (int h = 0; h < NH; ++h) {
  long orows[NRH];
  v4u pad[NRH], px[NRH], pz[NRH];
#pragma unroll
  for (int rr = 0; rr < NRH; ++rr) {
    const int m = mbase + (h * NRH + rr) * PPI + lane / LPR;
    const long orow = nok ? rowmap(a, m) : -1;
    orows[rr] = orow;
    const size_t off = (size_t)(orow < 0 ? 0 : orow) * a.ldo + n;
    pad[rr] = v4u{0u, 0u, 0u, 0u};
    px[rr] = v4u{0u, 0u, 0u, 0u};
    pz[rr] = v4u{0xffffffffu, 0xffffffffu, 0xffffffffu, 0xffffffffu};
    if (orow >= 0) {
      if (a.addend) {
        pad[rr] = *reinterpret_cast<const v4u*>(a.addend + off);
        if (a.addzm) pad[rr] &= mask8_to_and(a.addzm[off >> 3]);
      }
      if (bnw) {
        px[rr] = *reinterpret_cast<const v4u*>(a.bnx + off);
        if (a.bnzm) pz[rr] = mask8_to_bf(a.bnzm[off >> 3]);
        else if (a.bnz) pz[rr] = *reinterpret_cast<const v4u*>(a.bnz + off);
      }
    }
  }
#pragma unroll
  for (int i = 0; i < MIH; ++i)
#pragma unroll
    for (int j = 0; j < NI; ++j) {
      const int p = i * 16 + (lane & 15);
      const int g = j * 4 + (lane >> 4);
      *reinterpret_cast<v4f*>(wl + gpos(p, g)) = acc[h * MIH + i][j];
    }
  __builtin_amdgcn_s_waitcnt(0xc07f);
#pragma unroll
  for (int rr = 0; rr < NRH; ++rr) {
    const int r = rr;
    const int p = rr * PPI + lane / LPR;
    const v4f lo = *reinterpret_cast<const v4f*>(wl + gpos(p, 2 * q));
    const v4f hi = *reinterpret_cast<const v4f*>(wl + gpos(p, 2 * q + 1));
    const long orow = orows[r];
    if (orow >= 0 && a.out32) {
      float* o32 = a.out32 + (size_t)orow * a.ldo + n;
      v4f p0 = {lo[0] + bs[0], lo[1] + bs[1], lo[2] + bs[2], lo[3] + bs[3]};
      v4f p1 = {hi[0] + bs[4], hi[1] + bs[5], hi[2] + bs[6], hi[3] + bs[7]};
      if (a.accum32) {
        p0 += *reinterpret_cast<const v4f*>(o32);
        p1 += *reinterpret_cast<const v4f*>(o32 + 4);
      }
      *reinterpret_cast<v4f*>(o32) = p0;
      *reinterpret_cast<v4f*>(o32 + 4) = p1;
      continue;
    }
    if (orow >= 0) {
      float v[8] = {lo[0], lo[1], lo[2], lo[3], hi[0], hi[1], hi[2], hi[3]};
      if (a.addend) {
#pragma unroll
        for (int e = 0; e < 4; ++e) { v[2 * e] += lo_bf(pad[r][e]); v[2 * e + 1] += hi_bf(pad[r][e]); }
      }
      v4u o;
#pragma unroll
      for (int e = 0; e < 4; ++e) {
        float x0 = v[2 * e] + bs[2 * e], x1 = v[2 * e + 1] + bs[2 * e + 1];
        if (a.relu) { x0 = fmaxf(x0, 0.f); x1 = fmaxf(x1, 0.f); }
        o[e] = pack2bf(x0, x1);
      }
      if (a.stats) {
#pragma unroll
        for (int e = 0; e < 4; ++e) {
// ... 190 lines not shown
```

### csrc/conv_halo.hip

```cpp
#include <algorithm>
#include <cstdlib>
#include <type_traits>
#include <utility>

#include "common.h"
#include "kernels.h"
#include "conv_epilogue.h"

namespace {

__device__ __forceinline__ int hswz(int r) { return ((r >> 2) & 1) << 1; }

template <int W, int RB, int NIMG, int KT, int WPX>
struct HaloF {
  static constexpr int WP = W + 2;
  static constexpr int VR = NIMG * (RB + 1) - 1;
  static constexpr int VM = 16 * WPX;
  static constexpr int V = (VR * WP + VM - 1) / VM * VM;
  static constexpr int HR = NIMG * (RB + 1) + 1;
  static constexpr int XROWS = V + 2 * WP + 2;
  static constexpr int XI = (XROWS + 63) / 64;
  static constexpr int XR = XI * 64;
  static constexpr int XBYTES = XR * 64;
  static constexpr int WI = KT / 64;
// ... 589 lines not shown
  __syncthreads();

  constexpr int FM = SI_OW / 16;
  v4i acc[FM][4];
#pragma unroll
  for (int i = 0; i < FM; ++i)
#pragma unroll
    for (int j = 0; j < 4; ++j) acc[i][j] = v4i{0, 0, 0, 0};
  const int g = lane >> 4, col = lane & 15;
  const unsigned char* Wl = lds + SF_WOFF + col * SI_WST + g * 16;
#pragma unroll
  for (int st = 0; st < 4; ++st) {
    const int r = 2 * st + (g >> 1);
    const int t = 2 * wave + (r < 7 ? r : 6);
    const unsigned char* Pl = lds + SF_POFF + (t * SF_PW + 2 * col + 4 * (g & 1)) * 4;
    v4i fw[4], fx[FM];
#pragma unroll
    for (int j = 0; j < 4; ++j) fw[j] = *reinterpret_cast<const v4i*>(Wl + j * 16 * SI_WST + st * 64);
#pragma unroll
    for (int i = 0; i < FM; ++i) {
      const v2u lo = *reinterpret_cast<const v2u*>(Pl + i * 32 * 4), hi = *reinterpret_cast<const v2u*>(Pl + i * 32 * 4 + 8);
      fx[i] = v4i{(int)lo[0], (int)lo[1], (int)hi[0], (int)hi[1]};
    }
#pragma unroll
    for (int i = 0; i < FM; ++i)
#pragma unroll
      for (int j = 0; j < 4; ++j) acc[i][j] = __builtin_amdgcn_mfma_i32_16x16x64_i8(fw[j], fx[i], acc[i][j], 0, 0, 0);
  }
  const LinRowMap rm{((long)n * a.OH + oh0) * SI_OW};
  halo_epi_i8<FM, 4>(a, ep, acc, wave * SI_OW, 0, lane, rm);
}

int g_conv_halo = -1;

template <int W, int RB, int NIMG, int KT, int WPX>
void launch_halo_i8(const ConvArgs& a, const I8Epi& ep, hipStream_t st) {
  const int segs = a.Hs / RB;
  const int tiles_m = NIMG == 1 ? a.Nb * segs : (a.Nb + NIMG - 1) / NIMG;
  const int nwg = tiles_m * (a.Ncol / KT);
  conv_halo_kernel<W, RB, NIMG, KT, WPX, 3, 0, 1><<<dim3(nwg), dim3(256), 0, st>>>(a, ep);
}

}

extern "C" {

void bigdl_set_conv_halo(int v) { g_conv_halo = v; }

int bigdl_conv_halo_applies(const ConvArgs* a) {
  if (g_conv_halo < 0) {
    const char* e = getenv("BIGDL_CONV_HALO");
    g_conv_halo = e ? atoi(e) : 1;
  }
  if (!g_conv_halo || a->ntaps != 9 || a->mul_h != 1 || a->mul_w != 1 || !a->ident_out || a->out32 || a->pstride ||
      a->Hs != a->OH || a->Ws != a->OW || a->Hs != a->Ws || a->Kdim != 9 * a->Cs || (a->Cs % 32) ||
      (a->ldo % 8) || (a->Ncol % 8) || a->ldw < a->Kdim || (a->ldw % 8))
    return 0;
  const int W = a->Ws;
  const int kt = W == 56 ? 64 : 128;
  if (W != 56 && W != 28 && W != 14 && W != 7) return 0;
  const bool lean = a->addend == nullptr && (a->bnred == nullptr || a->stats != nullptr);
  if ((g_conv_halo == 2 && !lean) || (g_conv_halo == 3 && !lean && W == 56)) return 0;
  if (a->Ncol % kt) return 0;
  unsigned seen = 0;
  for (int t = 0; t < 9; ++t) {
    if (a->tap_h[t] < -1 || a->tap_h[t] > 1 || a->tap_w[t] < -1 || a->tap_w[t] > 1 || a->tap_k[t] < 0 ||
        a->tap_k[t] > 8)
      return 0;
    seen |= 1u << ((a->tap_h[t] + 1) * 3 + a->tap_w[t] + 1);
  }
  if (seen != 0x1ffu) return 0;
  if ((size_t)a->Nb * a->Hs * a->Ws * a->Cs * 2 >= (1ull << 31) - (1ull << 20)) return 0;
  if ((size_t)a->Ncol * a->ldw * 2 >= (1ull << 31)) return 0;
  const size_t M = (size_t)a->Nb * a->OH * a->OW;
  if (((M - 1) * (size_t)a->ldo + a->Ncol) * 2 >= 0x7ff00000ull) return 0;
  if (a->pre && (a->addend || (a->bnred && !a->stats) || a->Cs > PRE_MAXC || (g_conv_halo != 1 && g_conv_halo != 2)))
    return 0;
  auto al = [](const void* p) { return (reinterpret_cast<uintptr_t>(p) & 15) == 0; };
  return al(a->src) && al(a->wt) && al(a->out) && al(a->addend) && al(a->bnx) && al(a->bnz);
}

int bigdl_conv_halo(const ConvArgs* a, hipStream_t st) {
  switch (a->Ws) {
    case 56: launch_halo_f<56, 4, 1, 64, 4>(*a, st); break;
    case 28: launch_halo_f<28, 7, 1, 128, 2>(*a, st); break;
    case 14: launch_halo_f<14, 14, 1, 128, 2>(*a, st); break;
    case 7: launch_halo_f<7, 7, 3, 128, 2>(*a, st); break;
    default: return -1;
  }
  return 0;
}

int bigdl_conv_halo_i8_applies(const ConvArgs* a, const I8Epi* ep) {
  if (ep->add8 != nullptr || (a->Cs % 64) || (a->Ncol % 4) || (a->ldo % 4) || (a->ldw % 16)) return 0;
  if (g_conv_halo < 0) (void)bigdl_conv_halo_applies(a);
  if (!g_conv_halo) return 0;
  ConvArgs b = *a;
  b.addend = nullptr; b.bnred = nullptr; b.stats = nullptr;
  const int keep = g_conv_halo;
  g_conv_halo = 1;
  const int ok = bigdl_conv_halo_applies(&b);
  g_conv_halo = keep;
  return ok;
}

static int g_stem_i8 = -1;
// ... 42 lines not shown
```

### csrc/conv_igemm.hip

```cpp
#include "common.h"
#include "kernels.h"
#include <stdlib.h>

#include "conv_epilogue.h"


namespace {

constexpr int BK = 64;

__device__ __attribute__((aligned(64))) bf16_t g_zero_granule[32];
__device__ __forceinline__ v4u load16(const bf16_t* p, bool ok) {
  return *reinterpret_cast<const v4u*>(ok ? p : g_zero_granule);
}

template <int MI, int NI, int TM, int TN>
__device__ __forceinline__ void nt_epilogue(const ConvArgs& a, v4f (&acc)[MI][NI], int mbase, int nbase, int lane,
                                            int bid) {
  const int ohw = a.OH * a.OW;
  const bool vec_ok = (a.Ncol & 3) == 0 && (a.ldo & 3) == 0;
#pragma unroll
  for (int j = 0; j < NI; ++j) {
    const int nb = nbase + j * 16 + (lane >> 4) * 4;
    float bs[4] = {0.f, 0.f, 0.f, 0.f};
// ... 1509 lines not shown
      glds16(src, (LDS_PTR(void))(A + (j * 8 + wave) * 16 * BKS));
    }
#pragma unroll
    for (int j = 0; j < 2; ++j) {
      const bf16_t* src = bvalid[j] ? wrow[j] + wk : g_zero_granule;
      glds16(src, (LDS_PTR(void))(B + (j * 8 + wave) * 16 * BKS));
    }
  };
  const int foff = (lane & 15) * BKS + ((((lane >> 4) ^ ((lane >> 1) & 3))) << 3);

  v4f acc[MI][NI];
#pragma unroll
  for (int i = 0; i < MI; ++i)
#pragma unroll
    for (int j = 0; j < NI; ++j) acc[i][j] = v4f{0.f, 0.f, 0.f, 0.f};

  if (nk > 0) issue(kt0, 0);
  if (nk > 1) issue(kt0 + 1, 1);
  if (nk > 2) issue(kt0 + 2, 2);
  if (nk > 2) asm volatile("s_waitcnt vmcnt(%0)" ::"n"(2 * L) : "memory");
  else if (nk > 1) asm volatile("s_waitcnt vmcnt(%0)" ::"n"(L) : "memory");
  else asm volatile("s_waitcnt vmcnt(0)" ::: "memory");
  __builtin_amdgcn_s_barrier();
  for (int kt = 0; kt < nk; ++kt) {
    const int cur = kt & 3;
    if (kt + 3 < nk) issue(kt0 + kt + 3, (kt + 3) & 3);
    const bf16_t* A = lds + cur * STAGE;
    const bf16_t* B = A + BM * BKS;
    v8s fa[MI], fb[NI];
#pragma unroll
    for (int j = 0; j < NI; ++j) fb[j] = *reinterpret_cast<const v8s*>(B + (wn * TN + j * 16) * BKS + foff);
#pragma unroll
    for (int i = 0; i < MI; ++i) fa[i] = *reinterpret_cast<const v8s*>(A + (wm * TM + i * 16) * BKS + foff);
#pragma unroll
    for (int i = 0; i < MI; ++i)
#pragma unroll
      for (int j = 0; j < NI; ++j)
        acc[i][j] = __builtin_amdgcn_mfma_f32_16x16x32_bf16(fb[j], fa[i], acc[i][j], 0, 0, 0);
    const int ahead = min(nk - 1, kt + 3) - (kt + 1);
    if (ahead >= 2) asm volatile("s_waitcnt vmcnt(%0) lgkmcnt(0)" ::"n"(2 * L) : "memory");
    else if (ahead == 1) asm volatile("s_waitcnt vmcnt(%0) lgkmcnt(0)" ::"n"(L) : "memory");
    else asm volatile("s_waitcnt vmcnt(0) lgkmcnt(0)" ::: "memory");
    __builtin_amdgcn_s_barrier();
  }
  float* wl = reinterpret_cast<float*>(lds) + wave * SL;
  if constexpr (SPLIT) {
    store_partials_lds<MI, NI, TM, TN, NH>(a.ws + (size_t)blockIdx.y * a.M * a.Ncol, a.M, a.Ncol, acc,
                                           m0 + wm * TM, n0 + wn * TN, lane, wl);
  } else {
    nt_epilogue_lds<MI, NI, TM, TN, NH, WGN * SL, WGM>(a, acc, m0 + wm * TM, n0 + wn * TN, lane, bid, wl, wm);
  }
}

template <int BN, int NS, bool FASTK = true, int BM = 128, int ABN = 0>
__global__ __launch_bounds__(256, NS == 2 ? 4 : ((NS == 3 && BM == 128) ? 3 : 2)) void conv_nt_g4_kernel(ConvArgs a) {
  constexpr int BKS = 32;
  constexpr bool SHORTK = NS == 2;
  constexpr int WGM = 2, WGN = 2;
  constexpr int TM = BM / WGM, TN = BN / WGN;
  constexpr int MI = TM / 16, NI = TN / 16;
  constexpr int STAGE = (BM + BN) * BKS;
  constexpr int AI = BM / 64, BI = BN / 64;
  constexpr int L = AI + BI;
  constexpr int NH = BM == 256 ? 4 : (4 * TM * TN * 4 <= NS * STAGE * 2) ? 1 : 2;
  constexpr int SL = (TM / NH) * TN;
  static_assert(4 * SL * 4 <= NS * STAGE * 2, "epilogue chunk must fit the stages");
  __shared__ __attribute__((aligned(1024))) bf16_t lds[NS * STAGE + 3 * CONV_MAX_TAPS];
  short* taps = reinterpret_cast<short*>(lds + NS * STAGE);

  const int tid = threadIdx.x, lane = tid & 63;
  const int wave = __builtin_amdgcn_readfirstlane(tid >> 6);
  const int wm = wave / WGN, wn = wave % WGN;
  const int tiles_n = (a.Ncol + BN - 1) / BN;
  const int tiles_m = (a.M + BM - 1) / BM;
  const int nwg = tiles_m * tiles_n;
  const int bid = xcd_remap(blockIdx.x, nwg);
  const int tm = bid / tiles_n, tn = bid % tiles_n;
  const int m0 = tm * BM, n0 = tn * BN;
  const int nk = (a.Kdim + BKS - 1) / BKS;

  const int rsub = lane >> 2;
  const int gsrc = (lane & 3) ^ ((rsub >> 1) & 3);
  const int ps = a.pstride > 0 ? a.pstride : a.Cs;
  int a_pix[AI], a_h[AI], a_w[AI];
  const int ohw = a.OH * a.OW;
#pragma unroll
  for (int j = 0; j < AI; ++j) {
    const int m = m0 + (j * 4 + wave) * 16 + rsub;
    if (m < a.M) {
      const int nb = m / ohw, rem = m - nb * ohw;
      const int oh = rem / a.OW, ow = rem - oh * a.OW;
      a_pix[j] = nb * a.Hs * a.Ws;
      a_h[j] = oh * a.mul_h;
      a_w[j] = ow * a.mul_w;
    } else {
      a_pix[j] = 0; a_h[j] = -(1 << 28); a_w[j] = -(1 << 28);
    }
  }
  const bf16_t* wrow[BI];
  bool bvalid[BI];
#pragma unroll
  for (int j = 0; j < BI; ++j) {
    const int n = n0 + (j * 4 + wave) * 16 + rsub;
    bvalid[j] = n < a.Ncol;
    wrow[j] = a.wt + (size_t)(bvalid[j] ? n : 0) * a.ldw + (FASTK ? gsrc * 8 : 0);
  }
  if (tid < a.ntaps) {
// ... 43 lines not shown
#pragma unroll
  for (int i = 0; i < MI; ++i)
#pragma unroll
    for (int j = 0; j < NI; ++j) acc[i][j] = v4f{0.f, 0.f, 0.f, 0.f};

#pragma unroll
  for (int k = 0; k < (SHORTK ? 2 : NS - 1); ++k)
    if (k < nk) issue(k, k);
  {
    const int ahead = min(nk - 1, SHORTK ? 1 : NS - 2);
    if (ahead >= 2) asm volatile("s_waitcnt vmcnt(%0)" ::"n"(2 * L) : "memory");
    else if (ahead == 1) asm volatile("s_waitcnt vmcnt(%0)" ::"n"(L) : "memory");
    else asm volatile("s_waitcnt vmcnt(0)" ::: "memory");
  }
  __builtin_amdgcn_s_barrier();
  int cur = 0;
  for (int kt = 0; kt < nk; ++kt) {
    if (!SHORTK && kt + NS - 1 < nk) issue(kt + NS - 1, cur == 0 ? NS - 1 : cur - 1);
    const bf16_t* A = lds + cur * STAGE;
    const bf16_t* B = A + BM * BKS;
    v8s fa[MI], fb[NI];
#pragma unroll
    for (int j = 0; j < NI; ++j) fb[j] = *reinterpret_cast<const v8s*>(B + (wn * TN + j * 16) * BKS + foff);
#pragma unroll
    for (int i = 0; i < MI; ++i) fa[i] = *reinterpret_cast<const v8s*>(A + (wm * TM + i * 16) * BKS + foff);
    if constexpr (ABN) {
      const int c0 = (kt * BKS) % a.Cs + 8 * (lane >> 4);
      const v4f s0 = *reinterpret_cast<const v4f*>(a.pre + c0), s1 = *reinterpret_cast<const v4f*>(a.pre + c0 + 4);
      const v4f t0 = *reinterpret_cast<const v4f*>(a.pre + a.Cs + c0), t1 = *reinterpret_cast<const v4f*>(a.pre + a.Cs + c0 + 4);
      const float sc[8] = {s0[0], s0[1], s0[2], s0[3], s1[0], s1[1], s1[2], s1[3]};
      const float sh[8] = {t0[0], t0[1], t0[2], t0[3], t1[0], t1[1], t1[2], t1[3]};
#pragma unroll
      for (int i = 0; i < MI; ++i) {
        v4u u = __builtin_bit_cast(v4u, fa[i]);
#pragma unroll
        for (int e = 0; e < 4; ++e)
          u[e] = pack2bf(fmaxf(lo_bf(u[e]) * sc[2 * e] + sh[2 * e], 0.f), fmaxf(hi_bf(u[e]) * sc[2 * e + 1] + sh[2 * e + 1], 0.f));
        fa[i] = __builtin_bit_cast(v8s, u);
      }
    }
#pragma unroll
    for (int i = 0; i < MI; ++i)
#pragma unroll
      for (int j = 0; j < NI; ++j)
        acc[i][j] = __builtin_amdgcn_mfma_f32_16x16x32_bf16(fb[j], fa[i], acc[i][j], 0, 0, 0);
    const int ahead = min(nk - 1, kt + NS - 1) - (kt + 1);
    if (ahead >= 2) asm volatile("s_waitcnt vmcnt(%0) lgkmcnt(0)" ::"n"(2 * L) : "memory");
    else if (ahead == 1) asm volatile("s_waitcnt vmcnt(%0) lgkmcnt(0)" ::"n"(L) : "memory");
    else asm volatile("s_waitcnt vmcnt(0) lgkmcnt(0)" ::: "memory");
    __builtin_amdgcn_s_barrier();
    cur = cur == NS - 1 ? 0 : cur + 1;
  }
  float* wl = reinterpret_cast<float*>(lds) + wave * SL;
  nt_epilogue_lds<MI, NI, TM, TN, NH, WGN * SL, WGM>(a, acc, m0 + wm * TM, n0 + wn * TN, lane, bid, wl, wm);
}

template <bool SPLIT, int ABL = 0, bool SK = false>
__global__ __launch_bounds__(512, 2) void conv_nt_p8_kernel(ConvArgs a) {
  constexpr int BM = 256, BN = 256, BKT = 64;
  constexpr int WGM = 2, WGN = 4;
  constexpr int TM = BM / WGM, TN = BN / WGN;
  constexpr int MI = TM / 16, NI = TN / 16;
  constexpr int PIECE = 128 * BKT;
  constexpr int BUF = 4 * PIECE;
  constexpr int NH = 4;
  constexpr int SL = (TM / NH) * TN;
  static_assert(8 * SL * 4 <= 2 * BUF * 2, "epilogue chunk must fit the buffers");
  __shared__ __attribute__((aligned(1024))) bf16_t lds[2 * BUF + 3 * CONV_MAX_TAPS + 8];
  short* taps = reinterpret_cast<short*>(lds + 2 * BUF);
  int* skflag = reinterpret_cast<int*>(lds + 2 * BUF + 3 * CONV_MAX_TAPS);

  const int tid = threadIdx.x, lane = tid & 63;
  const int wave = __builtin_amdgcn_readfirstlane(tid >> 6);
  const int wm = wave / WGN, wn = wave % WGN;
  const int tiles_n = (a.Ncol + BN - 1) / BN;
  const int tiles_m = (a.M + BM - 1) / BM;
  const int nwg = tiles_m * tiles_n;
  constexpr bool KTAIL = (ABL & 64) != 0;
  const int nk_all = KTAIL ? (a.Kdim + BKT - 1) / BKT : a.Kdim / BKT;
  if (tid < a.ntaps) {
    taps[tid] = a.tap_h[tid];
    taps[CONV_MAX_TAPS + tid] = a.tap_w[tid];
    taps[2 * CONV_MAX_TAPS + tid] = a.tap_k[tid];
  }
  __syncthreads();

  const long I = (long)nwg * nk_all;
  const long G = gridDim.x;
  long it = SK ? ((long)blockIdx.x * I) / G : 0;
  const long it_end = SK ? ((long)(blockIdx.x + 1) * I) / G : 1;
  auto wg_of = [&](long x) -> int {
    long w = (x * G) / I;
    while (w + 1 < G && ((w + 1) * I) / G <= x) ++w;
    while (w > 0 && (w * I) / G > x) --w;
    return (int)w;
  };

  for (;;) {
  int bid, tm, tn, kt0, nk;
  if constexpr (SK) {
    if (it >= it_end) break;
    const int tile = (int)(it / nk_all);
    kt0 = (int)(it - (long)tile * nk_all);
    nk = (int)min((long)(nk_all - kt0), it_end - it);
    it += nk;
    bid = tile;
    tm = tile / tiles_n; tn = tile % tiles_n;
// ... 198 lines not shown
  } else {
    nt_epilogue_lds<MI, NI, TM, TN, NH, WGN * SL, WGM>(a, acc, m0 + wm * TM, n0 + wn * TN, lane, bid, wl, wm);
  }
  if constexpr (!SK) break;
  }
}

template <int K, int CG, int BMW, bool F32T, bool EXT, bool PRE = false>
__global__ __launch_bounds__(256, K >= 256 ? 1 : 2) void conv_nt_s1_kernel(ConvArgs a) {
  constexpr int KF = K / 32, MI = BMW / 16, PGN = 4 / CG, BM = BMW * PGN;
  constexpr bool PF = EXT && K >= 128;
  constexpr int NB = (EXT && K == 128) ? 2 : 3;
  constexpr int GPR = F32T ? 16 : 8;
  constexpr int NR = BMW / 8;
  __shared__ __attribute__((aligned(16))) unsigned lds[4 * BMW * GPR * 4 + (PRE ? 2 * K : 0)];
  const int lane = threadIdx.x & 63;
  const int wave = __builtin_amdgcn_readfirstlane(threadIdx.x >> 6);
  const int cg = wave % CG, pg = wave / CG;
  const int nchb = a.Ncol / (64 * CG);
  const int chb = blockIdx.x % nchb, wgi = blockIdx.x / nchb, ngr = gridDim.x / nchb;
  const int c0 = (chb * CG + cg) * 64;
  const int ntiles = (a.M + BM - 1) / BM;
  unsigned* wl = lds + wave * BMW * GPR * 4;
  const int q = lane & 7;
  const int n = c0 + 8 * q;

  v8s wf[4][KF];
#pragma unroll
  for (int j = 0; j < 4; ++j)
#pragma unroll
    for (int kk = 0; kk < KF; ++kk)
      wf[j][kk] = *reinterpret_cast<const v8s*>(a.wt + (size_t)(c0 + 16 * j + (lane & 15)) * a.ldw + 32 * kk +
                                                8 * (lane >> 4));
  const float* ptab = reinterpret_cast<const float*>(lds + 4 * BMW * GPR * 4);
  if constexpr (PRE) {
    for (int i = threadIdx.x; i < K / 2; i += 256)
      reinterpret_cast<v4f*>(lds + 4 * BMW * GPR * 4)[i] = reinterpret_cast<const v4f*>(a.pre)[i];
    __syncthreads();
  }
  float bs[8], bmu[8], bsc[8], bsh[8];
  const bool bnw = EXT && a.bnred && !a.stats;
#pragma unroll
  for (int e = 0; e < 8; ++e) {
    bs[e] = (F32T && a.bias) ? a.bias[n + e] : 0.f;
    bmu[e] = bnw ? a.bnmean[n + e] : 0.f;
    bsc[e] = (bnw && a.bnaff) ? a.bnaff[n + e] : 0.f;
    bsh[e] = (bnw && a.bnaff) ? a.bnaff[a.Ncol + n + e] : 0.f;
  }
  typedef float v2f __attribute__((ext_vector_type(2)));
  v2f p1[4], p2[4];
#pragma unroll
  for (int e = 0; e < 4; ++e) p1[e] = p2[e] = v2f{0.f, 0.f};
  const size_t ob = EXT ? ((size_t)(a.M - 1) * a.ldo + a.Ncol) * 2 : 0;
  const __amdgpu_buffer_rsrc_t r_add = rsrc_of(a.addend, (EXT && a.addend) ? ob : 0);
  const __amdgpu_buffer_rsrc_t r_azm = rsrc_of(a.addzm, (EXT && a.addzm) ? ob / 16 : 0);
  const __amdgpu_buffer_rsrc_t r_bx = rsrc_of(a.bnx, bnw ? ob : 0);
  const __amdgpu_buffer_rsrc_t r_bzm = rsrc_of(a.bnzm, (bnw && a.bnzm) ? ob / 16 : 0);
  const __amdgpu_buffer_rsrc_t r_out = rsrc_of(a.out, ob);
  const int zmode = !bnw ? 0 : a.bnzm ? 1 : a.bnaff ? 3 : 0;
  const bool azm = a.addzm != nullptr;

  auto load = [&](v8s (&af)[MI][KF], int t) {
    const int p0 = t * BM + pg * BMW;
#pragma unroll
    for (int i = 0; i < MI; ++i) {
      const int m = min(p0 + 16 * i + (lane & 15), a.M - 1);
#pragma unroll
      for (int kk = 0; kk < KF; ++kk)
        af[i][kk] = *reinterpret_cast<const v8s*>(a.src + (size_t)m * K + 32 * kk + 8 * (lane >> 4));
    }
  };

  struct ExtOps { v4u pad[EXT ? NR : 1], px[EXT ? NR : 1]; unsigned pza[EXT ? NR : 1], pzz[EXT ? NR : 1]; };
  auto load_ext = [&](ExtOps& e, int t) {
    if constexpr (EXT) {
      const int p0 = t * BM + pg * BMW;
#pragma unroll
      for (int rr = 0; rr < NR; ++rr) {
        const int m = min(p0 + rr * 8 + (lane >> 3), a.M - 1);
        const size_t off = (size_t)m * a.ldo + n;
        const unsigned eb = (unsigned)(off * 2), zo = (unsigned)(off >> 3);
        e.pad[rr] = __builtin_bit_cast(v4u, __builtin_amdgcn_raw_buffer_load_b128(r_add, eb, 0, 0));
        e.px[rr] = __builtin_bit_cast(v4u, __builtin_amdgcn_raw_buffer_load_b128(r_bx, eb, 0, 0));
        e.pza[rr] = __builtin_amdgcn_raw_buffer_load_b8(r_azm, zo, 0, 0);
        e.pzz[rr] = __builtin_amdgcn_raw_buffer_load_b8(r_bzm, zo, 0, 0);
      }
    }
  };

  auto compute_store = [&](v8s (&af)[MI][KF], ExtOps& eo, int t) {
    const int p0 = t * BM + pg * BMW;
    ExtOps el;
    if constexpr (EXT && !PF) load_ext(el, t);
    ExtOps& e = PF ? eo : el;
    auto& pad = e.pad;
    auto& px = e.px;
    v4f acc[MI][4];
#pragma unroll
    for (int i = 0; i < MI; ++i)
#pragma unroll
      for (int j = 0; j < 4; ++j) acc[i][j] = v4f{0.f, 0.f, 0.f, 0.f};
    if constexpr (PRE) {
#pragma unroll
      for (int kk = 0; kk < KF; ++kk) {
        const int c = 32 * kk + 8 * (lane >> 4);
        const v4f s0 = *reinterpret_cast<const v4f*>(ptab + c), s1 = *reinterpret_cast<const v4f*>(ptab + c + 4);
        const v4f b0 = *reinterpret_cast<const v4f*>(ptab + K + c), b1 = *reinterpret_cast<const v4f*>(ptab + K + c + 4);
        const float sc[8] = {s0[0], s0[1], s0[2], s0[3], s1[0], s1[1], s1[2], s1[3]};
        const float sh[8] = {b0[0], b0[1], b0[2], b0[3], b1[0], b1[1], b1[2], b1[3]};
#pragma unroll
        for (int i = 0; i < MI; ++i) {
          v4u u = __builtin_bit_cast(v4u, af[i][kk]);
#pragma unroll
          for (int e = 0; e < 4; ++e)
            u[e] = pack2bf(fmaxf(lo_bf(u[e]) * sc[2 * e] + sh[2 * e], 0.f),
                           fmaxf(hi_bf(u[e]) * sc[2 * e + 1] + sh[2 * e + 1], 0.f));
          af[i][kk] = __builtin_bit_cast(v8s, u);
        }
      }
    }
#pragma unroll
    for (int kk = 0; kk < KF; ++kk)
#pragma unroll
      for (int i = 0; i < MI; ++i)
#pragma unroll
        for (int j = 0; j < 4; ++j)
          acc[i][j] = __builtin_amdgcn_mfma_f32_16x16x32_bf16(wf[j][kk], af[i][kk], acc[i][j], 0, 0, 0);
#pragma unroll
    for (int i = 0; i < MI; ++i)
#pragma unroll
      for (int j = 0; j < 4; ++j) {
        const int p = 16 * i + (lane & 15), qq = lane >> 4;
        if constexpr (F32T) {
          const int g = 4 * j + qq;
          *reinterpret_cast<v4f*>(wl + (p * GPR + (g ^ (p & 15))) * 4) = acc[i][j];
// ... 136 lines not shown
  long rpb = (long)rpi * 8;
  long bx = (P + rpb - 1) / rpb;
  const long cap = 8192 / gy;
  if (bx > cap) {
    bx = cap;
    rpb = (P + bx - 1) / bx;
  }
  if (bx < 1) bx = 1;
  *rpb_out = rpb;
  return dim3((unsigned)bx, (unsigned)gy);
}

__global__ __launch_bounds__(256) void conv_splitk_epilogue_kernel(ConvArgs a, long rpb) {
  __shared__ float sm[256 * 16];
  const int G = a.Ncol >> 3;
  const int gbase = blockIdx.y * 256;
  const int gcount = min(256, G - gbase);
  const int rpi = 256 / gcount;
  const int g = gbase + threadIdx.x % gcount, rsub = threadIdx.x / gcount;
  const bool act = rsub < rpi;
  const long rbeg = blockIdx.x * rpb, rend = min((long)a.M, rbeg + rpb);
  const int n = g * 8;
  const size_t plane = (size_t)a.M * a.Ncol;
  const int ohw = a.OH * a.OW;
  float bs[8], bmu[8], bsc[8], bsh[8], s1[8], s2[8];
  const bool bnw = a.bnred && !a.stats;
#pragma unroll
  for (int e = 0; e < 8; ++e) {
    bs[e] = (act && a.bias) ? a.bias[n + e] : 0.f;
    bmu[e] = (act && bnw) ? a.bnmean[n + e] : 0.f;
    bsc[e] = (act && bnw && a.bnaff) ? a.bnaff[n + e] : 0.f;
    bsh[e] = (act && bnw && a.bnaff) ? a.bnaff[a.Ncol + n + e] : 0.f;
    s1[e] = s2[e] = 0.f;
  }
  if (act) {
    for (long m = rbeg + rsub; m < rend; m += rpi) {
      float v[8];
      const float* p = a.ws + (size_t)m * a.Ncol + n;
      {
        const v4f lo = *reinterpret_cast<const v4f*>(p), hi = *reinterpret_cast<const v4f*>(p + 4);
        v[0] = lo[0]; v[1] = lo[1]; v[2] = lo[2]; v[3] = lo[3]; v[4] = hi[0]; v[5] = hi[1]; v[6] = hi[2]; v[7] = hi[3];
      }
      for (int s = 1; s < a.ksplit; ++s) {
        const v4f lo = *reinterpret_cast<const v4f*>(p + s * plane), hi = *reinterpret_cast<const v4f*>(p + s * plane + 4);
        v[0] += lo[0]; v[1] += lo[1]; v[2] += lo[2]; v[3] += lo[3]; v[4] += hi[0]; v[5] += hi[1]; v[6] += hi[2]; v[7] += hi[3];
      }
      long orow = m;
      if (!a.ident_out) {
        const int nb = (int)(m / ohw), rem = (int)(m - (long)nb * ohw);
        const int oh = rem / a.OW, ow = rem - oh * a.OW;
        orow = ((long)nb * a.OHo + oh * a.omul_h + a.ooff_h) * a.OWo + ow * a.omul_w + a.ooff_w;
      }
      const size_t off = (size_t)orow * a.ldo + n;
      if (a.addend) {
        v4u q = *reinterpret_cast<const v4u*>(a.addend + off);
        if (a.addzm) q &= mask8_to_and(a.addzm[off >> 3]);
#pragma unroll
        for (int e = 0; e < 4; ++e) { v[2 * e] += lo_bf(q[e]); v[2 * e + 1] += hi_bf(q[e]); }
      }
      v4u o;
#pragma unroll
      for (int e = 0; e < 4; ++e) {
        float x0 = v[2 * e] + bs[2 * e], x1 = v[2 * e + 1] + bs[2 * e + 1];
        if (a.relu) { x0 = fmaxf(x0, 0.f); x1 = fmaxf(x1, 0.f); }
        o[e] = pack2bf(x0, x1);
      }
      if (a.stats) {
#pragma unroll
        for (int e = 0; e < 4; ++e) {
          const float y0 = lo_bf(o[e]), y1 = hi_bf(o[e]);
          s1[2 * e] += y0; s2[2 * e] += y0 * y0;
          s1[2 * e + 1] += y1; s2[2 * e + 1] += y1 * y1;
        }
      } else if (bnw) {
        const v4u px = *reinterpret_cast<const v4u*>(a.bnx + off);
        v4u pz = v4u{0xffffffffu, 0xffffffffu, 0xffffffffu, 0xffffffffu};
        if (a.bnzm) pz = mask8_to_bf(a.bnzm[off >> 3]);
        else if (a.bnz) pz = *reinterpret_cast<const v4u*>(a.bnz + off);
#pragma unroll
        for (int e = 0; e < 4; ++e) {
          float d0 = lo_bf(o[e]), d1 = hi_bf(o[e]);
          const float x0 = lo_bf(px[e]), x1 = hi_bf(px[e]);
          if (a.bnz || a.bnzm) {
            if (!(lo_bf(pz[e]) > 0.f)) d0 = 0.f;
            if (!(hi_bf(pz[e]) > 0.f)) d1 = 0.f;
          } else if (a.bnaff) {
            if (!(x0 * bsc[2 * e] + bsh[2 * e] > 0.f)) d0 = 0.f;
            if (!(x1 * bsc[2 * e + 1] + bsh[2 * e + 1] > 0.f)) d1 = 0.f;
          }
          s1[2 * e] += d0; s2[2 * e] += d0 * (x0 - bmu[2 * e]);
          s1[2 * e + 1] += d1; s2[2 * e + 1] += d1 * (x1 - bmu[2 * e + 1]);
        }
      }
      *reinterpret_cast<v4u*>(a.out + off) = o;
    }
  }
  float* const red = a.stats ? a.stats : a.bnred;
  if (red == nullptr) return;
#pragma unroll
  for (int e = 0; e < 8; ++e) { sm[threadIdx.x * 16 + e] = s1[e]; sm[threadIdx.x * 16 + 8 + e] = s2[e]; }
  __syncthreads();
  for (int w = threadIdx.x; w < gcount * 16; w += 256) {
    const int gg = w >> 4, slot = w & 15;
    float t = 0.f;
    for (int rs = 0; rs < rpi; ++rs) t += sm[(rs * gcount + gg) * 16 + slot];
    const int ch = (gbase + gg) * 8 + (slot & 7);
    atomicAdd(red + (size_t)(blockIdx.x & (BIGDL_STAT_SLOTS - 1)) * 2 * a.Ncol + (slot < 8 ? 0 : a.Ncol) + ch, t);
  }
// ... 97 lines not shown
  const long q = (tiles * nk) / G;
  if (q < 4) return 0;
  return (int)(nk / q + 2);
}

template <int BN, int NS, int BM = 128>
void launch_nt_g4(const ConvArgs& a, hipStream_t st) {
  const int nwg = ((a.M + BM - 1) / BM) * ((a.Ncol + BN - 1) / BN);
  static const int abn = [] { const char* e = getenv("BIGDL_G4_ABN"); return e ? atoi(e) : 0; }();
  if (abn && a.pre && BM == 128 && NS == 3 && a.Cs % 32 == 0)
    conv_nt_g4_kernel<BN, NS, true, BM, 1><<<dim3(nwg), dim3(256), 0, st>>>(a);
  else if (a.Cs % 32 == 0) conv_nt_g4_kernel<BN, NS, true, BM><<<dim3(nwg), dim3(256), 0, st>>>(a);
  else conv_nt_g4_kernel<BN, NS, false, BM><<<dim3(nwg), dim3(256), 0, st>>>(a);
}

int g_conv_g4 = -1;
static int g4_pick() {
  if (g_conv_g4 < 0) {
    const char* e = getenv("BIGDL_CONV_G4");
    g_conv_g4 = e ? atoi(e) : 3;
  }
  return g_conv_g4;
}

static bool g4_slowk() {
  static const int v = [] { const char* e = getenv("BIGDL_CONV_G4_SLOWK"); return e ? atoi(e) : 1; }();
  return v != 0;
}

int g_conv_shortk = -1;
static bool conv_shortk() {
  if (g_conv_shortk < 0) {
    const char* e = getenv("BIGDL_CONV_SHORTK");
    g_conv_shortk = e ? atoi(e) : 0;
  }
  return g_conv_shortk != 0;
}

int g_conv_s1 = -1;
static bool s1_applies(const ConvArgs* a) {
  if (g_conv_s1 < 0) {
    const char* e = getenv("BIGDL_CONV_S1");
    g_conv_s1 = e ? atoi(e) : 2;
  }
  if (!g_conv_s1 || a->out32 || !a->ident_out || a->ntaps != 1 || a->tap_h[0] || a->tap_w[0] || a->tap_k[0]) return false;
  if (a->mul_h != 1 || a->mul_w != 1 || a->Hs != a->OH || a->Ws != a->OW) return false;
  const bool ext = a->addend != nullptr || (a->bnred != nullptr && a->stats == nullptr);
  if ((a->Kdim != 64 && a->Kdim != 128 && !(a->Kdim == 256 && (g_conv_s1 == 2 || (g_conv_s1 == 3 && !ext)))) ||
      a->Cs != a->Kdim || (a->Ncol % 64) || (a->ldo % 8) || (a->ldw % 8))
    return false;
  if (((size_t)(a->M - 1) * a->ldo + a->Ncol) * 2 >= 0x7ff00000u) return false;
  if (a->bnred && !a->stats && a->bnz && !a->bnzm) return false;
  if (a->pre && (a->addend || (a->bnred && !a->stats))) return false;
  auto al = [](const void* p) { return (reinterpret_cast<uintptr_t>(p) & 15) == 0; };
  return al(a->src) && al(a->wt) && al(a->out) && al(a->addend) && al(a->bnx) && al(a->bnz);
}

template <int K, int CG, int BMW, bool F32T, bool EXT, bool PRE = false>
void launch_s1(const ConvArgs& a, hipStream_t st) {
  static int cus = 0;
  if (cus == 0) {
    int dev = 0;
    (void)hipGetDevice(&dev);
    (void)hipDeviceGetAttribute(&cus, hipDeviceAttributeMultiprocessorCount, dev);
    if (cus <= 0) cus = 256;
  }
  const int nchb = a.Ncol / (64 * CG);
  const int tiles = (a.M + BMW * (4 / CG) - 1) / (BMW * (4 / CG));
  constexpr int occ = K >= 256 ? 1 : 2;
  int per = std::max(1, (occ * cus) / nchb);
  per = std::min(per, tiles);
  conv_nt_s1_kernel<K, CG, BMW, F32T, EXT, PRE><<<dim3(per * nchb), dim3(256), 0, st>>>(a);
}

template <int K, int CG>
void launch_s1_cg(const ConvArgs& a, hipStream_t st) {
  const bool ext = a.addend != nullptr || (a.bnred != nullptr && a.stats == nullptr);
  const bool f32t = ext || a.bias != nullptr;
  if constexpr (K == 256) {
    if (a.pre && f32t) launch_s1<K, CG, 16, true, false, true>(a, st);
    else if (a.pre) launch_s1<K, CG, 16, false, false, true>(a, st);
    else if (ext) launch_s1<K, CG, 16, true, true>(a, st);
    else if (f32t) launch_s1<K, CG, 16, true, false>(a, st);
    else launch_s1<K, CG, 16, false, false>(a, st);
  } else {
  constexpr int BW = K == 64 ? 64 : 32;
  if (a.pre && f32t) launch_s1<K, CG, BW / 2, true, false, true>(a, st);
  else if (a.pre) launch_s1<K, CG, 32, false, false, true>(a, st);
  else if (ext) launch_s1<K, CG, BW / 2, true, true>(a, st);
  else if (f32t) launch_s1<K, CG, BW / 2, true, false>(a, st);
  else launch_s1<K, CG, BW, false, false>(a, st);
  }
}

static void launch_s1_any(const ConvArgs& a, hipStream_t st) {
  const int cg = (a.Ncol % 256 == 0) ? 4 : (a.Ncol % 128 == 0) ? 2 : 1;
  if (a.Kdim == 64) {
    if (cg == 4) launch_s1_cg<64, 4>(a, st);
    else if (cg == 2) launch_s1_cg<64, 2>(a, st);
    else launch_s1_cg<64, 1>(a, st);
  } else if (a.Kdim == 128) {
    if (cg == 4) launch_s1_cg<128, 4>(a, st);
    else if (cg == 2) launch_s1_cg<128, 2>(a, st);
    else launch_s1_cg<128, 1>(a, st);
  } else {
    if (cg == 4) launch_s1_cg<256, 4>(a, st);
    else if (cg == 2) launch_s1_cg<256, 2>(a, st);
    else launch_s1_cg<256, 1>(a, st);
  }
}

int g_conv_impl = -1;
int conv_impl() {
  if (g_conv_impl < 0) {
    const char* e = getenv("BIGDL_CONV_IMPL");
    g_conv_impl = e ? atoi(e) : 1;
  }
  return g_conv_impl;
}

}

extern "C" {

void bigdl_set_conv_impl(int impl) { g_conv_impl = impl; }
void bigdl_set_conv_s1(int v) { g_conv_s1 = v; }
void bigdl_set_conv_sk(int v) { g_conv_sk = v; }
void bigdl_set_conv_g4(int v) { g_conv_g4 = v; }
void bigdl_set_conv_shortk(int v) { g_conv_shortk = v; }
int g_wgrad_p8 = -1;
void bigdl_set_conv_p8(int v) { g_conv_p8 = v; }
void bigdl_set_wgrad_p8(int v) { g_wgrad_p8 = v; }
int bigdl_get_conv_g4() { return g4_pick(); }
int bigdl_get_conv_impl() { return conv_impl(); }

long bigdl_conv_nt_plan(ConvArgs* a) {
  a->ksplit = 0;
  if (a->Cs % 8 != 0 || a->M <= 0 || conv_impl() < 1) return 0;
  if (a->pstride > 0 && a->pstride != a->Cs) return 0;
  if (conv_impl() == 1 && s1_applies(a)) return 0;
  if (conv_impl() == 1 && bigdl_conv_halo_applies(a)) return 0;
  if (conv_impl() == 1 && bigdl_stem_fwd_applies(a)) return 0;
  if (g_conv_p8 < 0) (void)p8_pick(a);
  const int sk = sk_pick(a);
  if (sk > 0) {
    a->ksplit = -sk;
    const long tiles = (long)((a->M + 255) / 256) * ((a->Ncol + 255) / 256);
    return tiles * sk * 65536L + tiles;
  }
  const int p8 = conv_impl() == 1 ? p8_pick(a) : 0;
  if (p8 > 1) {
    a->ksplit = p8;
    return (long)p8 * a->M * a->Ncol;
  }
  if (p8 == 1) return 0;
  const int k = w8_pick(a);
  if (k > 1) {
    a->ksplit = k;
    return (long)k * a->M * a->Ncol;
  }
  return 0;
}

int bigdl_conv_pre_applies(const ConvArgs* a) {
  if (a->Cs % 8 != 0 || a->Kdim != a->ntaps * a->Cs || a->M <= 0 || a->pstride > 0 || conv_impl() != 1) return 0;
  if (bigdl_stem_fwd_applies(a)) return 0;
  return (s1_applies(a) || bigdl_conv_halo_applies(a)) ? 1 : 0;
}

int bigdl_conv_nt(const ConvArgs* a, hipStream_t st) {
  if (a->Cs % 8 != 0 || a->Kdim != a->ntaps * a->Cs || a->ntaps < 1 || a->ntaps > CONV_MAX_TAPS) return -1;
  if (a->pre) {
    if (!bigdl_conv_pre_applies(a)) return -5;
    if (s1_applies(a)) launch_s1_any(*a, st);
    else if (bigdl_conv_halo(a, st) != 0) return -5;
    HIP_LAUNCH_CHECK();
    return 0;
  }
  if (a->bnred && (a->stats || a->bnx == nullptr || a->bnmean == nullptr || (a->Ncol & 7) || (a->ldo & 7))) return -2;
  if (a->out32 && ((a->Ncol & 7) || (a->ldo & 7) || a->stats || a->bnred || a->relu || a->addend)) return -3;
  if (a->M <= 0) return 0;
  const bool fastk = (a->Cs % BK) == 0;
  const int impl = conv_impl();
  if (impl == 1 && bigdl_stem_fwd_applies(a) && bigdl_stem_fwd(a, st) == 0) {
    HIP_LAUNCH_CHECK();
    return 0;
  }
  if (a->pstride > 0 && a->pstride != a->Cs) {
    if ((a->Ncol & 7) || (a->ldo & 7) || a->out32 || a->ws || a->bnred || !(fastk || a->Kdim % 8 == 0)) return -4;
    if (a->Ncol <= 64) launch_nt_g4<64, 3>(*a, st);
    else launch_nt_g4<128, 3>(*a, st);
    HIP_LAUNCH_CHECK();
    return 0;
  }
  if (impl == 1 && s1_applies(a)) {
    launch_s1_any(*a, st);
    HIP_LAUNCH_CHECK();
    return 0;
  }
  if (impl == 1 && bigdl_conv_halo_applies(a) && bigdl_conv_halo(a, st) == 0) {
    HIP_LAUNCH_CHECK();
    return 0;
  }
  if (a->ksplit < 0 && a->ws != nullptr) {
    ConvArgs b = *a;
    b.ksplit = -a->ksplit;
    const long tiles = (long)((a->M + 255) / 256) * ((a->Ncol + 255) / 256);
    bigdl_fill_bytes(b.ws + tiles * b.ksplit * 65536L, 0, tiles * 4, st);
    const dim3 grid((unsigned)std::min<long>(sk_cus(), tiles * (a->Kdim / 64)));
    conv_nt_p8_kernel<false, 0, true><<<grid, dim3(512), 0, st>>>(b);
    HIP_LAUNCH_CHECK();
    return 0;
  }
  const long p3_tiles = (long)((a->M + 255) / 256) * ((a->Ncol + 127) / 128);
  const long tiles128 = (long)((a->M + 127) / 128) * ((a->Ncol + (a->Ncol <= 64 ? 63 : 127)) / (a->Ncol <= 64 ? 64 : 128));
  const bool aligned_out = (a->Ncol & 7) == 0 && (a->ldo & 7) == 0;
  static const bool p3auto = [] { const char* e = getenv("BIGDL_CONV_P3AUTO"); return e ? atoi(e) != 0 : true; }();
  const bool p3_pick = impl == 2 || (impl == 1 && p3auto && a->M <= 50176 && a->Kdim >= 1024);
  const int p8 = impl == 1 ? p8_pick(a) : 0;
  const int w8 = (impl == 1 && p8 == 0) ? w8_pick(a) : 0;
  const bool p8_ktail = (a->Cs % 64) != 0;
  if (p8 > 1 && a->ksplit == p8 && a->ws != nullptr) {
    const int nwg = ((a->M + 255) / 256) * ((a->Ncol + 255) / 256);
    if (p8_ktail) conv_nt_p8_kernel<true, 64><<<dim3(nwg, p8), dim3(512), 0, st>>>(*a);
    else conv_nt_p8_kernel<true><<<dim3(nwg, p8), dim3(512), 0, st>>>(*a);
    long rpb = 0;
    const dim3 grid = splitk_grid(a->M, a->Ncol, &rpb);
    conv_splitk_epilogue_kernel<<<grid, dim3(256), 0, st>>>(*a, rpb);
  } else if (p8 == 1) {
    const int nwg = ((a->M + 255) / 256) * ((a->Ncol + 255) / 256);
    static const int abl = [] { const char* e = getenv("BIGDL_P8_ABL"); return e ? atoi(e) : 0; }();
    switch (p8_ktail ? 64 : abl) {
      case 64: conv_nt_p8_kernel<false, 64><<<dim3(nwg), dim3(512), 0, st>>>(*a); break;
      case 1: conv_nt_p8_kernel<false, 1><<<dim3(nwg), dim3(512), 0, st>>>(*a); break;
      case 2: conv_nt_p8_kernel<false, 2><<<dim3(nwg), dim3(512), 0, st>>>(*a); break;
      case 4: conv_nt_p8_kernel<false, 4><<<dim3(nwg), dim3(512), 0, st>>>(*a); break;
      case 8: conv_nt_p8_kernel<false, 8><<<dim3(nwg), dim3(512), 0, st>>>(*a); break;
      case 16: conv_nt_p8_kernel<false, 16><<<dim3(nwg), dim3(512), 0, st>>>(*a); break;
      case 32: conv_nt_p8_kernel<false, 32><<<dim3(nwg), dim3(512), 0, st>>>(*a); break;
      case 10: conv_nt_p8_kernel<false, 10><<<dim3(nwg), dim3(512), 0, st>>>(*a); break;
      default: conv_nt_p8_kernel<false><<<dim3(nwg), dim3(512), 0, st>>>(*a);
    }
  } else if (w8 > 1 && a->ksplit == w8 && a->ws != nullptr) {
    const int nwg = ((a->M + 255) / 256) * ((a->Ncol + 255) / 256);
    conv_nt_w8_kernel<true><<<dim3(nwg, w8), dim3(512), 0, st>>>(*a);
    long rpb = 0;
    const dim3 grid = splitk_grid(a->M, a->Ncol, &rpb);
    conv_splitk_epilogue_kernel<<<grid, dim3(256), 0, st>>>(*a, rpb);
  } else if (w8 == 1) {
    const int nwg = ((a->M + 255) / 256) * ((a->Ncol + 255) / 256);
    conv_nt_w8_kernel<false><<<dim3(nwg), dim3(512), 0, st>>>(*a);
  } else if (impl == 1 && g4_pick() && aligned_out && (a->Cs % 32 == 0 || (g4_slowk() && a->Kdim % 8 == 0)) &&
             (g4_pick() == 5 || !(p3_pick && fastk && p3_tiles >= 256))) {
    const long tiles256 = (long)((a->M + 255) / 256) * ((a->Ncol + 127) / 128);
    if (a->Ncol > 64 && (g4_pick() == 7 || (g4_pick() == 6 && tiles256 >= 512))) {
      launch_nt_g4<128, 3, 256>(*a, st);
    } else if (conv_shortk() && fastk && a->Kdim <= 64 && a->Ncol <= 64) {
      launch_nt_g4<64, 2>(*a, st);
    } else if (g4_pick() != 4) {
      if (a->Ncol <= 64) launch_nt_g4<64, 3>(*a, st);
      else launch_nt_g4<128, 3>(*a, st);
    } else {
      if (a->Ncol <= 64) launch_nt_g4<64, 4>(*a, st);
      else launch_nt_g4<128, 4>(*a, st);
    }
  } else if (fastk && p3_pick && p3_tiles >= 256) {
    if (a->Ncol <= 64) launch_nt_p3<64, 8, 1>(*a, st);
    else launch_nt_p3<128, 4, 2>(*a, st);
  } else if (fastk && impl == 3 && aligned_out && tiles128 > 2 * 256) {
    if (a->Ncol <= 64) launch_nt_pers<128, 64, 2>(*a, st);
    else launch_nt_pers<128, 128, 2>(*a, st);
  } else if (fastk && impl >= 1 && a->Kdim == BK && aligned_out && conv_onestage()) {
    if (a->Ncol <= 64) launch_nt_glds<128, 64, 2, true, 1>(*a, st);
    else launch_nt_glds<128, 128, 2, true, 1>(*a, st);
  } else if (fastk && impl >= 1) {
    if (a->Ncol <= 64) launch_nt_glds<128, 64, 2>(*a, st);
    else launch_nt_glds<128, 128, 2>(*a, st);
  } else if (!fastk && impl >= 1 && glds_slowk()) {
    if (a->Ncol <= 64) launch_nt_glds<128, 64, 2, false>(*a, st);
    else launch_nt_glds<128, 128, 2, false>(*a, st);
  } else if (a->Ncol <= 64) {
    launch_nt<128, 64, 2>(*a, fastk, st);
  } else {
    launch_nt<128, 128, 2>(*a, fastk, st);
  }
  HIP_LAUNCH_CHECK();
  return 0;
}

static bool wgrad_prefers_atomic(const WgradArgs* a) {
  static const int on = [] { const char* e = getenv("BIGDL_WGRAD_ATOMIC"); return e ? atoi(e) : 1; }();
  if (bigdl_deterministic()) return false;
  return on == 2 || (on == 1 && a->Ncol <= 64 && a->Kdim > 256);
}

int g_wgrad_g3 = -1;
static bool wgrad_g3() {
  if (g_wgrad_g3 < 0) {
    const char* e = getenv("BIGDL_WGRAD_G3");
    g_wgrad_g3 = e ? atoi(e) : 0;
  }
// ... 190 lines not shown
```

### csrc/kernels.h

```cpp
#pragma once
#include <hip/hip_runtime.h>
#include <stdint.h>

#define CONV_MAX_TAPS 64
struct ConvArgs {
  const uint16_t* src;
  const uint16_t* wt;
  uint16_t* out;
  const float* bias;
  float* stats;
  const uint16_t* addend;
  const uint8_t* addzm;
  const uint16_t* bnx;
  const uint16_t* bnz;
  const uint8_t* bnzm;
  const float* bnmean;
  const float* bnaff;
  float* bnred;
  int Nb, Hs, Ws, Cs;
  int OH, OW;
  int mul_h, mul_w;
  int ntaps, ldw;
  int M, Ncol, Kdim, ldo;
  int OHo, OWo, omul_h, omul_w, ooff_h, ooff_w, ident_out;
  int relu;
  short tap_h[CONV_MAX_TAPS], tap_w[CONV_MAX_TAPS], tap_k[CONV_MAX_TAPS];
  float* out32;
  int accum32;
  float* ws;
  int ksplit;
  int pstride;
  const float* pre;
};

struct I8Epi {
  const float* xscale;
  float xs_const;
  const float* wscale;
  int out_mode;
  float out_inv;
  const int8_t* add8;
  float add_scale;
  long add_ld;
};

struct WgradArgs {
  const uint16_t* dy;
  const uint16_t* src;
  float* dw;
  float* dbias;
  int Nb, Hs, Ws, Cs, OH, OW, R, S;
  int sh, sw, ph, pw, dh, dwl;
  int M, Ncol, Kdim, ldy;
  int m_per_split;
  float* ws;
  int splits;
  float* det_ws;
  const float* pre;
};

extern "C" {
void bigdl_fill_bytes(void* ptr, int value, long bytes, hipStream_t st);
int bigdl_deterministic();
void bigdl_set_deterministic(int v);
#define BIGDL_DET_SLOTS 128
void bigdl_colsum_bf16_ld(const uint16_t* x, float* out, long P, int K, long ld, hipStream_t st,
                          float* det_ws = nullptr);
int bigdl_conv_pre_applies(const ConvArgs* a);
int bigdl_conv_nt(const ConvArgs* a, hipStream_t st);
int bigdl_conv_halo_applies(const ConvArgs* a);
int bigdl_conv_halo(const ConvArgs* a, hipStream_t st);
void bigdl_set_conv_halo(int v);
int bigdl_conv_halo_i8_applies(const ConvArgs* a, const I8Epi* ep);
int bigdl_conv_halo_i8(const ConvArgs* a, const I8Epi* ep, hipStream_t st);
int bigdl_stem_fwd_applies(const ConvArgs* a);
int bigdl_stem_fwd(const ConvArgs* a, hipStream_t st);
void bigdl_set_stem_fwd(int v);
long bigdl_stem_wgrad_plan(const WgradArgs* a);
int bigdl_stem_wgrad(const WgradArgs* a, hipStream_t st);
void bigdl_set_stem_wgrad(int v);
long bigdl_conv_nt_plan(ConvArgs* a);
int bigdl_bmm_nt(const uint16_t* A, const uint16_t* B, float* C, int batch, int M, int N, int K, long sa, long sb,
                 long sc, int lda, int ldb, int ldc, float alpha, int accum, hipStream_t st);
void bigdl_nchw_to_pairs(const float* x, uint16_t* y, int N, int C, int H, int W, int Hp, int Wp, int ph, int pw,
                         hipStream_t st);
void bigdl_pair_weight(const uint16_t* w, uint16_t* wp, int K, int C, int R, int S, const long* strides,
                       hipStream_t st);
void bigdl_pair_wgrad_add(const float* dwp, float* gw, int K, int C, int R, int S, const long* strides, float scale,
                          hipStream_t st);
int bigdl_conv_wgrad(const WgradArgs* a, hipStream_t st);
long bigdl_conv_wgrad_plan(WgradArgs* a);
void bigdl_transpose_krsc(const uint16_t* w, uint16_t* wt, int K, int RS, int C, hipStream_t st);
void bigdl_transpose_krsc_batched(const long* desc, int n, int total_tiles, hipStream_t st);

#define BIGDL_STAT_SLOTS 128
void bigdl_bn_stats(const uint16_t* x, float* stats, long P, int C, hipStream_t st);
void bigdl_bn_finalize(const float* stats, int nslots, const float* gamma, const float* beta, float* run_mean,
                       float* run_var, float* save_mean, float* save_invstd, float* scale, float* shift,
                       long P, int C, float eps, float momentum, int training, hipStream_t st);
void bigdl_bn_slot_reduce(const float* in, int nslots, int C, float* out, hipStream_t st);
void bigdl_bn_apply(const uint16_t* x, const float* scale, const float* shift, const uint16_t* res,
                    uint16_t* y, long P, int C, int relu, hipStream_t st, uint8_t* zm = nullptr);
void bigdl_bn_bwd_reduce(const uint16_t* dz, const uint16_t* z, const uint16_t* x, const float* mean,
                         float* red, long P, int C, const float* aff, hipStream_t st, const uint8_t* zm = nullptr);
void bigdl_bn_bwd_apply(const uint16_t* dz, const uint16_t* z, const uint16_t* x, const float* mean,
                        const float* invstd, const float* gamma, const float* red, int nslots, float* coef,
                        uint16_t* dx, uint16_t* dres, float* dgamma, float* dbeta, long P, int C, int training,
                        const float* aff, hipStream_t st, const uint8_t* zm = nullptr,
                        const uint16_t* x2 = nullptr, const float* mean2 = nullptr, float* red2 = nullptr);

void bigdl_relu_fwd(const uint16_t* x, uint16_t* y, long n, hipStream_t st);
void bigdl_spin_us(double us, int* done, hipStream_t st);
void bigdl_dgrad_fill(uint16_t* out, const uint16_t* add, long npix, int H, int W, int C, int sh, int sw, unsigned mask,
                      hipStream_t st);
void bigdl_relu_bwd(const uint16_t* dy, const uint16_t* y, uint16_t* dx, long n, hipStream_t st);
void bigdl_add_bf16(const uint16_t* a, const uint16_t* b, uint16_t* y, long n, hipStream_t st);
void bigdl_nchw_f32_to_nhwc_bf16(const float* x, uint16_t* y, int N, int C, int H, int W, int Cp,
                                 hipStream_t st);
void bigdl_cast_f32_bf16(const float* x, uint16_t* y, long n, hipStream_t st);
void bigdl_colsum_bf16(const uint16_t* x, float* out, long P, int K, hipStream_t st, float* det_ws = nullptr);
void bigdl_ones_col_pack(const uint16_t* x, uint16_t* xe, long M, int K, hipStream_t st);
void bigdl_ones_col_acc(const float* gw, float* gW, float* gB, long N, int K, float sW, float sB, hipStream_t st);
void bigdl_cast_bf16_f32(const uint16_t* x, float* y, long n, hipStream_t st);

void bigdl_maxpool_fwd(const uint16_t* x, uint16_t* y, uint8_t* idx, int N, int H, int W, int C, int OH,
                       int OW, int kh, int kw, int sh, int sw, int ph, int pw, hipStream_t st, const float* pre = nullptr);
int bigdl_maxpool_pre_applies(int N, int H, int W, int C, int OH, int OW, int kh, int kw, int sh, int sw);
int bigdl_stem_i8_applies(const ConvArgs* a, const I8Epi* ep);
void bigdl_set_stem_i8(int v);
int bigdl_stem_i8_f32(const ConvArgs* a, const I8Epi* ep, const float* img, int C, int W, float inv, hipStream_t st);
int bigdl_stem_i8(const ConvArgs* a, const I8Epi* ep, hipStream_t st);
void bigdl_split_reduce_f32(const float* ws, float* dw, long n, int splits, hipStream_t st);
int bigdl_maxpool_bwd_bnred_applies(int N, int H, int W, int C, int OH, int OW, int kh, int kw, int sh, int sw, int ph,
                                    int pw);
void bigdl_maxpool_bwd_bnred(const uint16_t* dy, const uint8_t* idx, uint16_t* dx, int N, int C, int OH, int OW,
                             const uint16_t* bx, const float* mean, const float* aff, const uint8_t* zm, float* red,
                             hipStream_t st);
void bigdl_maxpool_bwd(const uint16_t* dy, const uint8_t* idx, uint16_t* dx, int N, int H, int W, int C,
                       int OH, int OW, int kh, int kw, int sh, int sw, int ph, int pw, hipStream_t st);
void bigdl_avgpool_fwd(const uint16_t* x, uint16_t* y, int N, int H, int W, int C, int OH, int OW, int kh,
                       int kw, int sh, int sw, int ph, int pw, int count_pad, hipStream_t st);
void bigdl_avgpool_bwd(const uint16_t* dy, uint16_t* dx, int N, int H, int W, int C, int OH, int OW, int kh,
                       int kw, int sh, int sw, int ph, int pw, int count_pad, hipStream_t st);

void bigdl_softmax_xent(const uint16_t* logits_bf16, const float* logits_f32, const float* labels,
                        float* loss, uint16_t* dlogits_bf16, float* dlogits_f32, int B, int K,
                        float label_base, float grad_scale, hipStream_t st);

void bigdl_sgd_step(float* w, const float* g, float* mom, uint16_t* w16, long n, const float* lr_dev, float lr,
                    float wd, float momentum, float dampening, int nesterov, int first, const long* seg_off,
                    const float* seg_wd, int nseg, long base, hipStream_t st);
void bigdl_adam_step(float* w, const float* g, float* m, float* v, uint16_t* w16, long n, float lr,
                     float beta1, float beta2, float eps, float wd, float bc1, float bc2, hipStream_t st);
void bigdl_sumsq(const float* x, float* out, long n, hipStream_t st, float* det_ws = nullptr);
void bigdl_scale_f32(float* x, long n, const float* scale_dev, float scale, hipStream_t st);
// ... 192 lines not shown
```

Measured before the change: 11790 images/sec.

## Fuse shortcut BN affine into residual apply and compact strided shortcut dgrad

In projection residual blocks, the shortcut BatchNorm's affine step is deferred and applied inside the main BN apply kernel on the residual operand, which avoids a separate elementwise pass and its full-size output. The strided 1x1 shortcut conv's data gradient is computed at its compact resolution and passed as a subsampled addend into the next dgrad epilogue, so no strided zero-filled full-size gradient is written. Some BN finalize kernels also hoist their per-channel loads. This adds new kernel template variants and addend index arithmetic, plus fallback paths that rematerialize when layouts do not match.

```diff
diff --git a/bigdl_amd/nn/conv.py b/bigdl_amd/nn/conv.py
--- a/bigdl_amd/nn/conv.py
+++ b/bigdl_amd/nn/conv.py
@@ -264,6 +264,8 @@
             bn_src = getattr(input, "_bn_bwd", None) if (getattr(self, "_dgrad_bn_ok", False) or once) else None
             if bn_src is not None and not torch.is_tensor(bn_src[4]):
                 bn_src = bn_src[:4] + ((input if bn_src[4] else None),)
+            if squeeze or eh or ew:
+                self.__dict__.pop("_dgrad_compact", None)
             gi = self._dgrad_gpu(x, gy, ph, pw, None if (squeeze or eh or ew or self.format != "NCHW") else bn_src)
         else:
             gy = self._relu_mask(gy)
@@ -276,6 +278,11 @@
         if squeeze:
             gi = gi.squeeze(0)
         return self._fmt_out(gi)
+
+    def compact_dgrad_ok(self):
+        return (self.nGroup == 1 and self.format == "NCHW" and self.kernelH == 1 and self.kernelW == 1
+                and (self.strideH > 1 or self.strideW > 1) and self.padH == 0 and self.padW == 0
+                and not self.fuse_relu and type(self)._dgrad_gpu is SpatialConvolution._dgrad_gpu)
 
     def _relu_mask(self, gy):
         if not self.fuse_relu:
@@ -302,6 +309,13 @@
             addend_zm = None
             if isinstance(addend, tuple):
                 addend, addend_zm = addend
+            addend_stride = getattr(addend, "_addend_stride", None)
+            compact = self.__dict__.pop("_dgrad_compact", False)
+            if (compact and addend is None and bn_src is None and Cp == x.shape[1] and self.compact_dgrad_ok()
+                    and (ph, pw) == (0, 0)):
+                gi = cv.conv2d_dgrad(gy16, wt, (x.shape[0], Cp, gy16.shape[2], gy16.shape[3]), (1, 1), (0, 0))
+                gi._addend_stride = (self.strideH, self.strideW)
+                return gi
             if addend is not None and Cp != x.shape[1]:
                 raise RuntimeError("dgrad addend requires unpadded channels")
             bn = None
@@ -313,7 +327,8 @@
                 bn = {"x": bx, "z": bz, "zm": bzm, "mean": bmean, "aff": baff,
                       "red": bnops.new_stats(Cp, gy16.device)}
             gi = cv.conv2d_dgrad(gy16, wt, xs, (self.strideH, self.strideW), (ph, pw),
-                                 (self.dilationH, self.dilationW), addend=addend, bn=bn, addend_zm=addend_zm)
+                                 (self.dilationH, self.dilationW), addend=addend, bn=bn, addend_zm=addend_zm,
+                                 addend_stride=addend_stride)
             if Cp != x.shape[1]:
                 gi = gi[:, : x.shape[1]].contiguous(memory_format=CL)
             elif bn is not None and bn.get("done"):
diff --git a/bigdl_amd/nn/fusion.py b/bigdl_amd/nn/fusion.py
--- a/bigdl_amd/nn/fusion.py
+++ b/bigdl_amd/nn/fusion.py
@@ -208,16 +208,45 @@
         a._defer_ok = True
 
 
+SHORTCUT_BN_FUSE = [os.environ.get("BIGDL_SHORTCUT_BN_FUSE", "1") != "0"]
+
+
+def _bn_plain_gpu_training(m):
+    return (isinstance(m, BatchNormalization) and m.train and m.sync_fn is None and m.dataFormat == "NCHW"
+            and m.nOutput % 8 == 0)
+
+
+def _qualifies(t):
+    return (torch.is_tensor(t) and t.is_cuda and t.dim() == 4 and t.dtype == torch.bfloat16
+            and t.is_contiguous(memory_format=torch.channels_last) and getattr(t, "_bn_pre", None) is None)
+
+
 def residual_forward(seq, x):
+    from ..ops import bn as bnops
+
     branch, short, bn = seq._residual_plan
     concat, add, relu = seq.modules
-    res = short.forward(x)
+    sbn = short.modules[-1] if isinstance(short, Sequential) and short.modules else None
+    if (SHORTCUT_BN_FUSE[0] and sbn is not None and short._residual_plan is None and _bn_plain_gpu_training(bn)
+            and _bn_plain_gpu_training(sbn) and not sbn.fuse_relu and sbn.nOutput == bn.nOutput
+            and torch.is_tensor(x) and x.is_cuda):
+        sbn._affine_defer = True
+    try:
+        res = short.forward(x)
+    finally:
+        if sbn is not None:
+            sbn.__dict__.pop("_affine_defer", None)
     h = x
     for m in branch.modules[:-1]:
         h = m.forward(h)
     if tuple(res.shape) != tuple(h.shape[:1]) + (bn.nOutput,) + tuple(h.shape[2:]):
         raise ValueError(f"residual block: shortcut output {tuple(res.shape)} does not match the branch output")
-    out = bn.updateOutput(h, residual=res)
+    aff2 = getattr(res, "_bn_aff", None)
+    if aff2 is not None and not (_qualifies(h) and h.stride() == res.stride()):
+        res = bnops.materialize(res)
+        sbn.output = short.output = res
+        aff2 = None
+    out = bn.updateOutput(h, residual=res, residual_aff=aff2)
     bn.output = out
     branch.output = out
     concat.output = Table(out, res)
@@ -231,6 +260,9 @@
 
 
 SHORTCUT_BN_RED = [os.environ.get("BIGDL_SHORTCUT_BN_RED", "1") != "0"]
+
+
+SHORTCUT_COMPACT = [os.environ.get("BIGDL_SHORTCUT_COMPACT", "1") != "0"]
 
 
 def _native_det():
@@ -271,9 +303,21 @@
         dh, dres = bn.backward_fused(seq._res_h, gradOutput, need_dres=True, sec=sec)
         if sec is not None:
             dres._bn_red = (sbn, sec[2])
-        gs = short.backward(x, dres)
+        sc0 = short.modules[0] if isinstance(short, Sequential) and short.modules else None
+        if (SHORTCUT_COMPACT[0] and can_fold and isinstance(sc0, SpatialConvolution) and sc0.compact_dgrad_ok()
+                and type(first)._dgrad_gpu is SpatialConvolution._dgrad_gpu and first.strideH == 1
+                and first.strideW == 1 and torch.is_tensor(x) and x.is_cuda and x.dim() == 4
+                and x.dtype == torch.bfloat16 and x.shape[1] == first.nInputPlane
+                and first.nOutputPlane % 32 == 0):
+            sc0._dgrad_compact = True
+        try:
+            gs = short.backward(x, dres)
+        finally:
+            if sc0 is not None:
+                sc0.__dict__.pop("_dgrad_compact", None)
     bn.gradInput = dh
-    fold = masked is not None or (can_fold and gs is not None and gs.dtype == x.dtype and gs.shape == x.shape)
+    fold = masked is not None or (can_fold and gs is not None and gs.dtype == x.dtype
+                                  and (gs.shape == x.shape or getattr(gs, "_addend_stride", None) is not None))
     g = dh
     for i in range(len(mods) - 2, -1, -1):
         inp = mods[i - 1].output if i > 0 else x
diff --git a/bigdl_amd/nn/normalization.py b/bigdl_amd/nn/normalization.py
--- a/bigdl_amd/nn/normalization.py
+++ b/bigdl_amd/nn/normalization.py
@@ -89,7 +89,7 @@
                 x = x.to(BF16).contiguous()
         return x
 
-    def updateOutput(self, input, residual=None):
+    def updateOutput(self, input, residual=None, residual_aff=None):
         if residual is None:
             residual = self.__dict__.pop("_graph_residual", None)
         x = self._to_nchw(input)
@@ -97,6 +97,8 @@
             stats = getattr(input, "_bn_stats", None) if self.train else None
             x = self._prep_gpu(x)
             res = residual
+            if residual_aff is not None and (res is None or res.dtype != BF16 or res.stride() != x.stride()):
+                raise ValueError("BatchNormalization: residual_aff needs a bf16 residual laid out like the input")
             if res is not None and (res.dtype != BF16 or res.stride() != x.stride()):
                 res = res.to(BF16).contiguous(memory_format=CL if x.dim() == 4 else torch.contiguous_format)
             zm = None
@@ -111,10 +113,18 @@
                 y = bnops.deferred(x, aff)
                 y._bn_bwd = (self, x, sm, aff, False)
                 return y
+            if (self.__dict__.pop("_affine_defer", False) and self.train and not self.fuse_relu and res is None
+                    and self.sync_fn is None and x.dim() == 4 and self.dataFormat == "NCHW" and x is input
+                    and getattr(input, "_bn_pre", None) is None):
+                sm, si, aff = bnops.bn_prepare_gpu(x, self.weight, self.bias, self.runningMean, self.runningVar,
+                                                   self.eps, self.momentum, stats=stats)
+                self.saveMean, self.saveStd = sm, si
+                self._aff, self._zm, self._xin = None, None, x
+                return bnops.deferred_affine(x, aff)
             y, sm, si, aff = bnops.bn_forward_gpu(x, self.weight, self.bias, self.runningMean, self.runningVar,
                                                    self.eps, self.momentum, self.train, stats=stats, res=res,
                                                    relu=self.fuse_relu, sync_fn=self.sync_fn if self.train else None,
-                                                   zm=zm)
+                                                   zm=zm, res_aff=residual_aff)
             self.saveMean, self.saveStd = sm, si
             self._aff = aff if (self.fuse_relu and res is None) else None
             self._zm = zm
@@ -122,6 +132,8 @@
             if self.train and self.fuse_relu:
                 y._bn_bwd = (self, x, sm, self._aff, zm if zm is not None else res is not None)
             return self._from_nchw(y)
+        if residual_aff is not None:
+            raise ValueError("BatchNormalization: residual_aff is a GPU-path operand")
         xf = x.float()
         y, mean, invstd = bnops.bn_forward_cpu(xf, self.weight, self.bias, self.runningMean, self.runningVar, self.eps,
                                                self.momentum, self.train,
diff --git a/bigdl_amd/ops/bn.py b/bigdl_amd/ops/bn.py
--- a/bigdl_amd/ops/bn.py
+++ b/bigdl_amd/ops/bn.py
@@ -59,7 +59,7 @@
 
 
 def bn_forward_gpu(x, gamma, beta, rmean, rvar, eps, momentum, training, stats=None, res=None, relu=False,
-                   out=None, sync_fn=None, zm=None):
+                   out=None, sync_fn=None, zm=None, res_aff=None):
     C = x.shape[1]
     P = _P(x)
     C_ = native.get()
@@ -82,7 +82,7 @@
         stats, nslots = scale, 0
     C_.bn_finalize(stats, nslots, gamma, beta, rmean, rvar, smean, sinv, scale, shift, Ptot, C, float(eps),
                    float(momentum), bool(training))
-    C_.bn_apply(x, scale, shift, res, out, P, C, bool(relu), zm)
+    C_.bn_apply(x, scale, shift, res, out, P, C, bool(relu), zm, res_aff)
     return out, smean, sinv, aff
 
 
@@ -111,13 +111,21 @@
     return y
 
 
+def deferred_affine(x, aff):
+    y = x.detach()
+    y._bn_aff = aff
+    return y
+
+
 def materialize(t):
-    aff = getattr(t, "_bn_pre", None)
+    aff, relu = getattr(t, "_bn_pre", None), True
+    if aff is None:
+        aff, relu = getattr(t, "_bn_aff", None), False
     if aff is None:
         return t
     C = t.shape[1]
     y = torch.empty_like(t)
-    native.get().bn_apply(t, aff[:C], aff[C:], None, y, _P(t), C, True)
+    native.get().bn_apply(t, aff[:C], aff[C:], None, y, _P(t), C, relu)
     return y
 
 
diff --git a/bigdl_amd/ops/conv.py b/bigdl_amd/ops/conv.py
--- a/bigdl_amd/ops/conv.py
+++ b/bigdl_amd/ops/conv.py
@@ -132,7 +132,8 @@
     return res
 
 
-def conv2d_dgrad(dy, w16t, x_shape, stride, pad, dil=(1, 1), out=None, addend=None, bn=None, addend_zm=None):
+def conv2d_dgrad(dy, w16t, x_shape, stride, pad, dil=(1, 1), out=None, addend=None, bn=None, addend_zm=None,
+                 addend_stride=None):
     N, C, H, W = x_shape
     _, K, OH, OW = dy.shape
     R, S = w16t.shape[1], w16t.shape[2]
@@ -144,6 +145,15 @@
         out = torch.empty((N, C, H, W), dtype=BF16, device=dy.device, memory_format=CL)
     if addend_zm is not None and (addend is None or covered != H * W):
         raise ValueError("conv2d_dgrad: a masked addend needs an addend and a data gradient that covers every pixel")
+    astr = []
+    if addend_stride is not None:
+        ash, asw = addend_stride
+        if addend_zm is not None:
+            raise ValueError("conv2d_dgrad: a subsampled addend takes no mask")
+        if addend is None or covered != H * W or C % 8 or tuple(addend.shape) != (N, C, -(-H // ash), -(-W // asw)):
+            raise ValueError("conv2d_dgrad: a subsampled addend is [N, C, ceil(H / ash), ceil(W / asw)], C % 8 == 0, "
+                             "on a data gradient that covers every pixel")
+        astr = [int(ash), int(asw)]
     if covered != H * W:
         mask = 0
         for (a, b, _, _, _) in phases:
@@ -165,7 +175,8 @@
         bn["done"] = True
     for (a, b, nI, nJ, taps) in phases:
         geo = [N, OH, OW, K, nI, nJ, 1, 1, ldw, C, C, H, W, stride[0], stride[1], a, b]
-        C_.conv_nt(dy, w16t, out, None, None, geo, taps, False, addend, addend_zm=addend_zm, **bnk)
+        C_.conv_nt(dy, w16t, out, None, None, geo, taps, False, addend, addend_zm=addend_zm, addend_stride=astr,
+                   **bnk)
     return out
 
 
diff --git a/csrc/batchnorm.hip b/csrc/batchnorm.hip
--- a/csrc/batchnorm.hip
+++ b/csrc/batchnorm.hip
@@ -126,6 +126,12 @@
   const int lane = threadIdx.x & 63, sl = lane & 31;
   const int c = (blockIdx.x * (blockDim.x >> 6) + (threadIdx.x >> 6)) * 2 + (lane >> 5);
   if (c >= C) return;
+  float g = 1.f, b = 0.f, rm = 0.f, rv = 1.f;
+  if (sl == 0) {
+    if (gamma) g = gamma[c];
+    if (beta) b = beta[c];
+    if (run_mean) { rm = run_mean[c]; rv = run_var[c]; }
+  }
   float mean, invstd;
   if (training) {
     double s1, s2;
@@ -138,25 +144,29 @@
     save_invstd[c] = invstd;
     if (run_mean) {
       const float unbiased = P > 1 ? var * (float)P / (float)(P - 1) : var;
-      run_mean[c] = momentum * mean + (1.f - momentum) * run_mean[c];
-      run_var[c] = momentum * unbiased + (1.f - momentum) * run_var[c];
+      run_mean[c] = momentum * mean + (1.f - momentum) * rm;
+      run_var[c] = momentum * unbiased + (1.f - momentum) * rv;
     }
   } else {
     if (sl != 0) return;
-    mean = run_mean[c];
-    invstd = rsqrtf(run_var[c] + eps);
+    mean = rm;
+    invstd = rsqrtf(rv + eps);
     if (save_mean) { save_mean[c] = mean; save_invstd[c] = invstd; }
   }
-  const float g = gamma ? gamma[c] : 1.f, b = beta ? beta[c] : 0.f;
   scale[c] = g * invstd;
   shift[c] = b - mean * g * invstd;
 }
 
-template <int U>
+__device__ __forceinline__ void load8(const float* p, float* v) {
+  const v4f a = *reinterpret_cast<const v4f*>(p), b = *reinterpret_cast<const v4f*>(p + 4);
+  v[0] = a[0]; v[1] = a[1]; v[2] = a[2]; v[3] = a[3]; v[4] = b[0]; v[5] = b[1]; v[6] = b[2]; v[7] = b[3];
+}
+
+template <int U, bool RA>
 __global__ __launch_bounds__(256) void bn_apply_kernel(const bf16_t* __restrict__ x, const float* __restrict__ scale,
                                                        const float* __restrict__ shift, const bf16_t* __restrict__ res,
                                                        bf16_t* __restrict__ y, long P, int C, long rpb, int relu,
-                                                       uint8_t* __restrict__ zm) {
+                                                       uint8_t* __restrict__ zm, const float* __restrict__ raff) {
   const int G = C >> 3;
   const int gbase = blockIdx.y * 256;
   const int gcount = min(256, G - gbase);
@@ -169,6 +179,11 @@
   const v4f b0 = *reinterpret_cast<const v4f*>(shift + c0), b1 = *reinterpret_cast<const v4f*>(shift + c0 + 4);
   const float sc[8] = {s0[0], s0[1], s0[2], s0[3], s1[0], s1[1], s1[2], s1[3]};
   const float sh[8] = {b0[0], b0[1], b0[2], b0[3], b1[0], b1[1], b1[2], b1[3]};
+  float rsc[8], rsh[8];
+  if (RA) {
+    load8(raff + c0, rsc);
+    load8(raff + C + c0, rsh);
+  }
   for (long r0 = rbeg + rsub; r0 < rend; r0 += (long)U * rpi) {
     v4u vx[U], vr[U];
 #pragma unroll
@@ -187,7 +202,16 @@
       for (int e = 0; e < 4; ++e) {
         float l = lo_bf(vx[u][e]) * sc[2 * e] + sh[2 * e];
         float h = hi_bf(vx[u][e]) * sc[2 * e + 1] + sh[2 * e + 1];
-        if (res) { l += lo_bf(vr[u][e]); h += hi_bf(vr[u][e]); }
+        if (res) {
+          unsigned q = vr[u][e];
+          if (RA) {
+            const float rl = lo_bf(q) * rsc[2 * e] + rsh[2 * e];
+            const float rh = hi_bf(q) * rsc[2 * e + 1] + rsh[2 * e + 1];
+            q = pack2bf(rl, rh);
+          }
+          l += lo_bf(q);
+          h += hi_bf(q);
+        }
         if (relu) { l = fmaxf(l, 0.f); h = fmaxf(h, 0.f); }
         o[e] = pack2bf(l, h);
       }
@@ -205,19 +229,27 @@
   const int lane = threadIdx.x & 63, sl = lane & 31;
   const int c = (blockIdx.x * (blockDim.x >> 6) + (threadIdx.x >> 6)) * 2 + (lane >> 5);
   if (c >= C) return;
+  float is = 0.f, g = 1.f, mu = 0.f, dg = 0.f, db = 0.f;
+  if (sl == 0) {
+    is = invstd[c];
+    if (gamma) g = gamma[c];
+    if (training) {
+      mu = mean[c];
+      if (dgamma) dg = dgamma[c];
+      if (dbeta) db = dbeta[c];
+    }
+  }
   double sdy = 0.0, sdyx = 0.0;
   if (training) slot_sums(red, nslots, C, c, sl, sdy, sdyx);
   if (sl != 0) return;
-  const float is = invstd[c];
-  const float g = gamma ? gamma[c] : 1.f;
   float A = g * is, B = 0.f, D = 0.f;
   if (training) {
     const float mdy = (float)(sdy / (double)P);
     const float mdyx = (float)(sdyx / (double)P) * is;
     B = -g * is * is * mdyx;
-    D = g * is * (mean[c] * is * mdyx - mdy);
-    if (dgamma) dgamma[c] += (float)sdyx * is;
-    if (dbeta) dbeta[c] += (float)sdy;
+    D = g * is * (mu * is * mdyx - mdy);
+    if (dgamma) dgamma[c] = dg + (float)sdyx * is;
+    if (dbeta) dbeta[c] = db + (float)sdy;
   }
   coef[c] = A; coef[C + c] = B; coef[2 * C + c] = D;
 }
@@ -228,11 +260,6 @@
   float t = 0.f;
   for (int k = 0; k < nslots; ++k) t += in[(size_t)k * 2 * C + c];
   out[c] = t;
-}
-
-__device__ __forceinline__ void load8(const float* p, float* v) {
-  const v4f a = *reinterpret_cast<const v4f*>(p), b = *reinterpret_cast<const v4f*>(p + 4);
-  v[0] = a[0]; v[1] = a[1]; v[2] = a[2]; v[3] = a[3]; v[4] = b[0]; v[5] = b[1]; v[6] = b[2]; v[7] = b[3];
 }
 
 template <int U, bool R2>
@@ -395,15 +422,21 @@
 }
 
 void bigdl_bn_apply(const uint16_t* x, const float* scale, const float* shift, const uint16_t* res, uint16_t* y,
-                    long P, int C, int relu, hipStream_t st, uint8_t* zm) {
+                    long P, int C, int relu, hipStream_t st, uint8_t* zm, const float* raff) {
   long rpb = 0;
   const dim3 grid = stationary_grid(P, C, &rpb);
+#define BN_APPLY(UU)                                                                                        \
+  if (raff && res)                                                                                          \
+    bn_apply_kernel<UU, true><<<grid, 256, 0, st>>>(x, scale, shift, res, y, P, C, rpb, relu, zm, raff);    \
+  else                                                                                                      \
+    bn_apply_kernel<UU, false><<<grid, 256, 0, st>>>(x, scale, shift, res, y, P, C, rpb, relu, zm, nullptr)
   switch (bn_unroll()) {
-    case 1: bn_apply_kernel<1><<<grid, 256, 0, st>>>(x, scale, shift, res, y, P, C, rpb, relu, zm); break;
-    case 2: bn_apply_kernel<2><<<grid, 256, 0, st>>>(x, scale, shift, res, y, P, C, rpb, relu, zm); break;
-    case 8: bn_apply_kernel<8><<<grid, 256, 0, st>>>(x, scale, shift, res, y, P, C, rpb, relu, zm); break;
-    default: bn_apply_kernel<4><<<grid, 256, 0, st>>>(x, scale, shift, res, y, P, C, rpb, relu, zm); break;
-  }
+    case 1: BN_APPLY(1); break;
+    case 2: BN_APPLY(2); break;
+    case 8: BN_APPLY(8); break;
+    default: BN_APPLY(4); break;
+  }
+#undef BN_APPLY
   HIP_LAUNCH_CHECK();
 }
 
diff --git a/csrc/bindings.cpp b/csrc/bindings.cpp
--- a/csrc/bindings.cpp
+++ b/csrc/bindings.cpp
@@ -33,7 +33,7 @@
 OptT conv_nt(const Tensor& src, const Tensor& wt, const Tensor& out, const OptT& bias, const OptT& stats,
              std::vector<int64_t> geo, std::vector<int64_t> taps, bool relu, const OptT& addend, const OptT& bn_x,
              const OptT& bn_z, const OptT& bn_mean, const OptT& bn_aff, const OptT& bn_red, bool accumulate,
-             const OptT& bn_zm, const OptT& addend_zm, const OptT& pre) {
+             const OptT& bn_zm, const OptT& addend_zm, const OptT& pre, std::vector<int64_t> addend_stride) {
   TORCH_CHECK(geo.size() == 17 || geo.size() == 18, "conv_nt: bad geometry");
   if (stats && stats->defined())
     TORCH_CHECK(stats->numel() >= BIGDL_STAT_SLOTS * 2 * geo[9], "conv_nt: stats must hold STAT_SLOTS x 2Ncol");
@@ -47,7 +47,9 @@
   else a.out = mbf(out, "out");
   a.bias = ocf(bias, "bias"); a.stats = omf(stats, "stats");
   a.addend = ocbf(addend, "addend");
-  if (a.addend) TORCH_CHECK(addend->numel() == out.numel(), "conv_nt: addend must match out");
+  const bool add_sub = !addend_stride.empty();
+  TORCH_CHECK(!add_sub || (a.addend && addend_stride.size() == 2), "conv_nt: addend_stride = (ash, asw) of an addend");
+  if (a.addend && !add_sub) TORCH_CHECK(addend->numel() == out.numel(), "conv_nt: addend must match out");
   a.bnx = ocbf(bn_x, "bn_x"); a.bnz = ocbf(bn_z, "bn_z"); a.bnmean = ocf(bn_mean, "bn_mean");
   a.bnaff = ocf(bn_aff, "bn_aff"); a.bnred = omf(bn_red, "bn_red");
   a.addzm = nullptr;
@@ -100,6 +102,12 @@
   TORCH_CHECK(a.ldo >= a.Ncol && out_avail >= ((int64_t)a.Nb * a.OHo * a.OWo - 1) * a.ldo + a.Ncol,
               "conv_nt: out too small");
   if (a.addend) TORCH_CHECK(a.ldo == a.Ncol, "conv_nt: an addend needs a dense output (ldo == Ncol)");
+  if (add_sub) {
+    const long rows = bigdl_conv_addend_grid(&a, (int)addend_stride[0], (int)addend_stride[1]);
+    TORCH_CHECK(rows > 0 && addend->numel() == rows * a.Ncol && (a.Ncol & 7) == 0,
+                "conv_nt: a subsampled addend is a dense [Nb][ceil(OHo / ash)][ceil(OWo / asw)][Ncol] tensor, Ncol % 8 "
+                "== 0, without a mask");
+  }
   TORCH_CHECK((a.OH - 1) * a.omul_h + a.ooff_h < a.OHo && (a.OW - 1) * a.omul_w + a.ooff_w < a.OWo,
               "conv_nt: output placement out of range");
   OptT materialised;
@@ -199,10 +207,15 @@
   bigdl_bn_slot_reduce(cf(in, "in"), (int)nslots, (int)C, mf(out, "out"), stream());
 }
 void bn_apply(const Tensor& x, const Tensor& scale, const Tensor& shift, const OptT& res, const Tensor& y, int64_t P,
-              int64_t C, bool relu, const OptT& zm) {
+              int64_t C, bool relu, const OptT& zm, const OptT& res_aff) {
   TORCH_CHECK(C % 8 == 0 && x.numel() == P * C && y.numel() == P * C, "bn_apply: shape");
+  const bool has_res = res && res->defined();
+  if (has_res) TORCH_CHECK(res->numel() == P * C, "bn_apply: res shape");
+  if (res_aff && res_aff->defined())
+    TORCH_CHECK(has_res && res_aff->numel() >= 2 * C && res_aff->is_contiguous(),
+                "bn_apply: res_aff is [2C] and needs res");
   bigdl_bn_apply(cbf(x, "x"), cf(scale, "scale"), cf(shift, "shift"), ocbf(res, "res"), mbf(y, "y"), P, (int)C,
-                 relu ? 1 : 0, stream(), omzm(zm, P, C, "zm"));
+                 relu ? 1 : 0, stream(), omzm(zm, P, C, "zm"), ocf(res_aff, "res_aff"));
 }
 void bn_bwd_reduce(const Tensor& dz, const OptT& z, const Tensor& x, const Tensor& mean, const Tensor& red, int64_t P,
                    int64_t C, const OptT& aff, const OptT& zm) {
@@ -1383,14 +1396,16 @@
         py::arg("geo"), py::arg("taps"), py::arg("relu"), py::arg("addend") = py::none(), py::arg("bn_x") = py::none(),
         py::arg("bn_z") = py::none(), py::arg("bn_mean") = py::none(), py::arg("bn_aff") = py::none(),
         py::arg("bn_red") = py::none(), py::arg("accumulate") = false, py::arg("bn_zm") = py::none(),
-        py::arg("addend_zm") = py::none(), py::arg("pre") = py::none());
+        py::arg("addend_zm") = py::none(), py::arg("pre") = py::none(),
+        py::arg("addend_stride") = std::vector<int64_t>());
+  m.def("conv_nt_last_path", &bigdl_conv_nt_last_path);
   m.def("conv_wgrad", &conv_wgrad, py::arg("dy"), py::arg("src"), py::arg("dw"), py::arg("dbias"), py::arg("geo"),
         py::arg("pre") = py::none());
   m.def("transpose_krsc", &transpose_krsc);
   m.def("bn_stats", &bn_stats);
   m.def("bn_finalize", &bn_finalize);
   m.def("bn_apply", &bn_apply, py::arg("x"), py::arg("scale"), py::arg("shift"), py::arg("res"), py::arg("y"),
-        py::arg("P"), py::arg("C"), py::arg("relu"), py::arg("zm") = py::none());
+        py::arg("P"), py::arg("C"), py::arg("relu"), py::arg("zm") = py::none(), py::arg("res_aff") = py::none());
   m.def("bn_slot_reduce", &bn_slot_reduce);
   m.attr("STAT_SLOTS") = BIGDL_STAT_SLOTS;
   m.def("bn_bwd_reduce", &bn_bwd_reduce, py::arg("dz"), py::arg("z"), py::arg("x"), py::arg("mean"), py::arg("red"),
diff --git a/csrc/conv_epilogue.h b/csrc/conv_epilogue.h
--- a/csrc/conv_epilogue.h
+++ b/csrc/conv_epilogue.h
@@ -15,7 +15,22 @@
   }
 };
 
-template <int MI, int NI, int TM, int TN, int NH = 1, int PAIR = 0, int NWM = 2, class RowMap = GemmRowMap>
+__device__ __forceinline__ unsigned recip_div(unsigned n, unsigned mg, int sh) {
+  return (unsigned)(((unsigned long long)n * mg) >> sh);
+}
+
+__device__ __forceinline__ long addend_row(const ConvArgs& a, long orow) {
+  if (a.ash == 0) return orow;
+  const unsigned r = (unsigned)orow;
+  const unsigned nb = recip_div(r, a.amg[0], a.amsh[0]), rem = r - nb * (unsigned)(a.OHo * a.OWo);
+  const unsigned h = recip_div(rem, a.amg[1], a.amsh[1]), w = rem - h * (unsigned)a.OWo;
+  const unsigned hq = recip_div(h, a.amg[2], a.amsh[2]), wq = recip_div(w, a.amg[3], a.amsh[3]);
+  const bool on = hq * (unsigned)a.ash == h && wq * (unsigned)a.asw == w;
+  return on ? ((long)nb * a.AH + hq) * a.AW + wq : -1;
+}
+
+template <int MI, int NI, int TM, int TN, int NH = 1, int PAIR = 0, int NWM = 2, class RowMap = GemmRowMap,
+          bool ASUB = false>
 __device__ __forceinline__ void nt_epilogue_lds(const ConvArgs& a, v4f (&acc)[MI][NI], int mbase, int nbase,
                                                 int lane, int bid, float* wl, int wm = 0, RowMap rowmap = {}) {
   constexpr int GR = TN / 4;
@@ -59,7 +74,12 @@
     pz[rr] = v4u{0xffffffffu, 0xffffffffu, 0xffffffffu, 0xffffffffu};
     if (orow >= 0) {
       if (a.addend) {
-        pad[rr] = *reinterpret_cast<const v4u*>(a.addend + off);
+        if constexpr (ASUB) {
+          const long ar = addend_row(a, orow);
+          if (ar >= 0) pad[rr] = *reinterpret_cast<const v4u*>(a.addend + (size_t)ar * a.ldo + n);
+        } else {
+          pad[rr] = *reinterpret_cast<const v4u*>(a.addend + off);
+        }
         if (a.addzm) pad[rr] &= mask8_to_and(a.addzm[off >> 3]);
       }
       if (bnw) {
diff --git a/csrc/conv_halo.hip b/csrc/conv_halo.hip
--- a/csrc/conv_halo.hip
+++ b/csrc/conv_halo.hip
@@ -665,6 +665,7 @@
     const char* e = getenv("BIGDL_CONV_HALO");
     g_conv_halo = e ? atoi(e) : 1;
   }
+  if (a->ash) return 0;
   if (!g_conv_halo || a->ntaps != 9 || a->mul_h != 1 || a->mul_w != 1 || !a->ident_out || a->out32 || a->pstride ||
       a->Hs != a->OH || a->Ws != a->OW || a->Hs != a->Ws || a->Kdim != 9 * a->Cs || (a->Cs % 32) ||
       (a->ldo % 8) || (a->Ncol % 8) || a->ldw < a->Kdim || (a->ldw % 8))
diff --git a/csrc/conv_igemm.hip b/csrc/conv_igemm.hip
--- a/csrc/conv_igemm.hip
+++ b/csrc/conv_igemm.hip
@@ -1585,7 +1585,7 @@
   }
 }
 
-template <int BN, int NS, bool FASTK = true, int BM = 128, int ABN = 0>
+template <int BN, int NS, bool FASTK = true, int BM = 128, int ABN = 0, bool ASUB = false>
 __global__ __launch_bounds__(256, NS == 2 ? 4 : ((NS == 3 && BM == 128) ? 3 : 2)) void conv_nt_g4_kernel(ConvArgs a) {
   constexpr int BKS = 32;
   constexpr bool SHORTK = NS == 2;
@@ -1735,7 +1735,8 @@
     cur = cur == NS - 1 ? 0 : cur + 1;
   }
   float* wl = reinterpret_cast<float*>(lds) + wave * SL;
-  nt_epilogue_lds<MI, NI, TM, TN, NH, WGN * SL, WGM>(a, acc, m0 + wm * TM, n0 + wn * TN, lane, bid, wl, wm);
+  nt_epilogue_lds<MI, NI, TM, TN, NH, WGN * SL, WGM, GemmRowMap, ASUB>(a, acc, m0 + wm * TM, n0 + wn * TN, lane, bid,
+                                                                       wl, wm);
 }
 
 template <bool SPLIT, int ABL = 0, bool SK = false>
@@ -2040,7 +2041,8 @@
 #pragma unroll
   for (int e = 0; e < 4; ++e) p1[e] = p2[e] = v2f{0.f, 0.f};
   const size_t ob = EXT ? ((size_t)(a.M - 1) * a.ldo + a.Ncol) * 2 : 0;
-  const __amdgpu_buffer_rsrc_t r_add = rsrc_of(a.addend, (EXT && a.addend) ? ob : 0);
+  const size_t ab = (EXT && K >= 128 && a.ash) ? ((size_t)((long)a.Nb * a.AH * a.AW - 1) * a.ldo + a.Ncol) * 2 : ob;
+  const __amdgpu_buffer_rsrc_t r_add = rsrc_of(a.addend, (EXT && a.addend) ? ab : 0);
   const __amdgpu_buffer_rsrc_t r_azm = rsrc_of(a.addzm, (EXT && a.addzm) ? ob / 16 : 0);
   const __amdgpu_buffer_rsrc_t r_bx = rsrc_of(a.bnx, bnw ? ob : 0);
   const __amdgpu_buffer_rsrc_t r_bzm = rsrc_of(a.bnzm, (bnw && a.bnzm) ? ob / 16 : 0);
@@ -2068,7 +2070,14 @@
         const int m = min(p0 + rr * 8 + (lane >> 3), a.M - 1);
         const size_t off = (size_t)m * a.ldo + n;
         const unsigned eb = (unsigned)(off * 2), zo = (unsigned)(off >> 3);
-        e.pad[rr] = __builtin_bit_cast(v4u, __builtin_amdgcn_raw_buffer_load_b128(r_add, eb, 0, 0));
+        unsigned ea = eb;
+        if constexpr (K >= 128) {
+          if (a.ash) {
+            const long ar = addend_row(a, m);
+            ea = ar >= 0 ? (unsigned)(((size_t)ar * a.ldo + n) * 2) : EOOB;
+          }
+        }
+        e.pad[rr] = __builtin_bit_cast(v4u, __builtin_amdgcn_raw_buffer_load_b128(r_add, ea, 0, 0));
         e.px[rr] = __builtin_bit_cast(v4u, __builtin_amdgcn_raw_buffer_load_b128(r_bx, eb, 0, 0));
         e.pza[rr] = __builtin_amdgcn_raw_buffer_load_b8(r_azm, zo, 0, 0);
         e.pzz[rr] = __builtin_amdgcn_raw_buffer_load_b8(r_bzm, zo, 0, 0);
@@ -2311,8 +2320,9 @@
         orow = ((long)nb * a.OHo + oh * a.omul_h + a.ooff_h) * a.OWo + ow * a.omul_w + a.ooff_w;
       }
       const size_t off = (size_t)orow * a.ldo + n;
-      if (a.addend) {
-        v4u q = *reinterpret_cast<const v4u*>(a.addend + off);
+      const long arow = a.addend ? addend_row(a, orow) : -1;
+      if (arow >= 0) {
+        v4u q = *reinterpret_cast<const v4u*>(a.addend + (size_t)arow * a.ldo + n);
         if (a.addzm) q &= mask8_to_and(a.addzm[off >> 3]);
 #pragma unroll
         for (int e = 0; e < 4; ++e) { v[2 * e] += lo_bf(q[e]); v[2 * e + 1] += hi_bf(q[e]); }
@@ -2516,6 +2526,7 @@
   if (((size_t)(a->M - 1) * a->ldo + a->Ncol) * 2 >= 0x7ff00000u) return false;
   if (a->bnred && !a->stats && a->bnz && !a->bnzm) return false;
   if (a->pre && (a->addend || (a->bnred && !a->stats))) return false;
+  if (a->ash && a->Kdim < 128) return false;
   auto al = [](const void* p) { return (reinterpret_cast<uintptr_t>(p) & 15) == 0; };
   return al(a->src) && al(a->wt) && al(a->out) && al(a->addend) && al(a->bnx) && al(a->bnz);
 }
@@ -2588,6 +2599,23 @@
 extern "C" {
 
 void bigdl_set_conv_impl(int impl) { g_conv_impl = impl; }
+static int g_last_path = 0;
+int bigdl_conv_nt_last_path() { return g_last_path; }
+
+long bigdl_conv_addend_grid(ConvArgs* a, int ash, int asw) {
+  const long rows = (long)a->Nb * a->OHo * a->OWo;
+  if (ash < 1 || asw < 1 || a->addzm || a->ldo != a->Ncol || rows <= 0 || rows >= (1L << 31)) return -1;
+  a->ash = ash; a->asw = asw;
+  a->AH = (a->OHo + ash - 1) / ash; a->AW = (a->OWo + asw - 1) / asw;
+  const unsigned d[4] = {(unsigned)(a->OHo * a->OWo), (unsigned)a->OWo, (unsigned)ash, (unsigned)asw};
+  for (int i = 0; i < 4; ++i) {
+    int l = 0;
+    while ((1ull << l) < d[i]) ++l;
+    a->amsh[i] = 31 + l;
+    a->amg[i] = (unsigned)(((1ull << (31 + l)) + d[i] - 1) / d[i]);
+  }
+  return (long)a->Nb * a->AH * a->AW;
+}
 void bigdl_set_conv_s1(int v) { g_conv_s1 = v; }
 void bigdl_set_conv_sk(int v) { g_conv_sk = v; }
 void bigdl_set_conv_g4(int v) { g_conv_g4 = v; }
@@ -2606,7 +2634,7 @@
   if (conv_impl() == 1 && bigdl_conv_halo_applies(a)) return 0;
   if (conv_impl() == 1 && bigdl_stem_fwd_applies(a)) return 0;
   if (g_conv_p8 < 0) (void)p8_pick(a);
-  const int sk = sk_pick(a);
+  const int sk = a->ash ? 0 : sk_pick(a);
   if (sk > 0) {
     a->ksplit = -sk;
     const long tiles = (long)((a->M + 255) / 256) * ((a->Ncol + 255) / 256);
@@ -2636,6 +2664,7 @@
   if (a->Cs % 8 != 0 || a->Kdim != a->ntaps * a->Cs || a->ntaps < 1 || a->ntaps > CONV_MAX_TAPS) return -1;
   if (a->pre) {
     if (!bigdl_conv_pre_applies(a)) return -5;
+    g_last_path = s1_applies(a) ? 1 : 2;
     if (s1_applies(a)) launch_s1_any(*a, st);
     else if (bigdl_conv_halo(a, st) != 0) return -5;
     HIP_LAUNCH_CHECK();
@@ -2647,6 +2676,7 @@
   const bool fastk = (a->Cs % BK) == 0;
   const int impl = conv_impl();
   if (impl == 1 && bigdl_stem_fwd_applies(a) && bigdl_stem_fwd(a, st) == 0) {
+    g_last_path = 5;
     HIP_LAUNCH_CHECK();
     return 0;
   }
@@ -2658,11 +2688,22 @@
     return 0;
   }
   if (impl == 1 && s1_applies(a)) {
+    g_last_path = 1;
     launch_s1_any(*a, st);
     HIP_LAUNCH_CHECK();
     return 0;
   }
   if (impl == 1 && bigdl_conv_halo_applies(a) && bigdl_conv_halo(a, st) == 0) {
+    g_last_path = 2;
+    HIP_LAUNCH_CHECK();
+    return 0;
+  }
+  g_last_path = 4;
+  if (a->ash && !(a->ksplit > 1 && a->ws != nullptr)) {
+    if ((a->Cs % 32) || (a->Ncol & 7) || (a->ldo & 7) || a->out32) return -6;
+    const int nwg = ((a->M + 127) / 128) * ((a->Ncol + (a->Ncol <= 64 ? 63 : 127)) / (a->Ncol <= 64 ? 64 : 128));
+    if (a->Ncol <= 64) conv_nt_g4_kernel<64, 3, true, 128, 0, true><<<dim3(nwg), dim3(256), 0, st>>>(*a);
+    else conv_nt_g4_kernel<128, 3, true, 128, 0, true><<<dim3(nwg), dim3(256), 0, st>>>(*a);
     HIP_LAUNCH_CHECK();
     return 0;
   }
@@ -2691,6 +2732,7 @@
     long rpb = 0;
     const dim3 grid = splitk_grid(a->M, a->Ncol, &rpb);
     conv_splitk_epilogue_kernel<<<grid, dim3(256), 0, st>>>(*a, rpb);
+    g_last_path = 3;
   } else if (p8 == 1) {
     const int nwg = ((a->M + 255) / 256) * ((a->Ncol + 255) / 256);
     static const int abl = [] { const char* e = getenv("BIGDL_P8_ABL"); return e ? atoi(e) : 0; }();
@@ -2711,6 +2753,7 @@
     long rpb = 0;
     const dim3 grid = splitk_grid(a->M, a->Ncol, &rpb);
     conv_splitk_epilogue_kernel<<<grid, dim3(256), 0, st>>>(*a, rpb);
+    g_last_path = 3;
   } else if (w8 == 1) {
     const int nwg = ((a->M + 255) / 256) * ((a->Ncol + 255) / 256);
     conv_nt_w8_kernel<false><<<dim3(nwg), dim3(512), 0, st>>>(*a);
diff --git a/csrc/kernels.h b/csrc/kernels.h
--- a/csrc/kernels.h
+++ b/csrc/kernels.h
@@ -31,6 +31,9 @@
   int ksplit;
   int pstride;
   const float* pre;
+  int ash = 0, asw = 0, AH = 0, AW = 0;
+  unsigned amg[4] = {0, 0, 0, 0};
+  int amsh[4] = {0, 0, 0, 0};
 };
 
 struct I8Epi {
@@ -68,6 +71,8 @@
                           float* det_ws = nullptr);
 int bigdl_conv_pre_applies(const ConvArgs* a);
 int bigdl_conv_nt(const ConvArgs* a, hipStream_t st);
+long bigdl_conv_addend_grid(ConvArgs* a, int ash, int asw);
+int bigdl_conv_nt_last_path();
 int bigdl_conv_halo_applies(const ConvArgs* a);
 int bigdl_conv_halo(const ConvArgs* a, hipStream_t st);
 void bigdl_set_conv_halo(int v);
@@ -100,7 +105,8 @@
                        long P, int C, float eps, float momentum, int training, hipStream_t st);
 void bigdl_bn_slot_reduce(const float* in, int nslots, int C, float* out, hipStream_t st);
 void bigdl_bn_apply(const uint16_t* x, const float* scale, const float* shift, const uint16_t* res,
-                    uint16_t* y, long P, int C, int relu, hipStream_t st, uint8_t* zm = nullptr);
+                    uint16_t* y, long P, int C, int relu, hipStream_t st, uint8_t* zm = nullptr,
+                    const float* res_aff = nullptr);
 void bigdl_bn_bwd_reduce(const uint16_t* dz, const uint16_t* z, const uint16_t* x, const float* mean,
                          float* red, long P, int C, const float* aff, hipStream_t st, const uint8_t* zm = nullptr);
 void bigdl_bn_bwd_apply(const uint16_t* dz, const uint16_t* z, const uint16_t* x, const float* mean,
```

Result: faster. 11990 images/sec, median of 6 (+1.7%).
